# QueensGambit/CrazyAra

Measured on AMD Instinct MI355X. Metric: nn_evals_per_sec, higher is better.
Workload: dtype f16x3; 1 GPU; crazyhouse RISEv2 19-block (34x8x8 planes -> 5184 policy + value), batch=256, inputs resident in HBM, random-init seeded weights; batch=256, parallelism=replicas x1, precision=float16x3

## Files before the change

crazyara_amd/csrc/nn/kernels.h:

```cpp
#pragma once
#include <hip/hip_runtime.h>
#include <cstdint>

namespace cra {

typedef _Float16 half_t;

constexpr int kSquares = 64;

inline int64_t packed_weight_elems(int cout_pad, int k_total) { return int64_t(cout_pad) * k_total; }

struct ConvArgs {
    const void* x;
    const void* wpk;
    const void* wpk_lo;
    const float* bias;
    const void* resid;
    void* out;
    int batch;
    int cin;
    int cout_pad;
    int cout_real;
    int cout_ld;
    int ks;
    int relu;
    int out_policy_f32;
    int out_flat;
    int flat_pitch;
    int out_rows_f32;
    int rows_valid;
    float* softmax_out;
    const float* planes;
    int planes_c;
    int p8;
    float acc_scale;
    const void *pre_wpk, *pre_wpk_lo;
    const float* pre_bias;
    float pre_acc_scale;
    int dev;
    int few_boards;
    int x_ld;
};

template <typename T> void launch_conv_gemm(const ConvArgs& a, hipStream_t s);

struct BlockArgs {
    const void* x;
    void* y;
    const void* w1pk;
    const float* b1;
    const float* wdw;
    const float* b2;
    const void* w3pk;
    const void* w1pk_lo;
    const void* w3pk_lo;
    const float* b3;
    int batch, C, cop_pad, ks;
    const float* gate;
    float* pool_out;
    const float* dwpk;
};
template <typename T> void launch_block(const BlockArgs& a, hipStream_t s);
void launch_conv_gemm_x3(const ConvArgs& a, hipStream_t s);
void launch_block_x3(const BlockArgs& a, hipStream_t s);
void init_x3_kernel_attributes();
int block_x3_chunk_channels();
struct X3TowerBlock {
    const void *w1pk, *w1pk_lo, *w3pk, *w3pk_lo;
    const float* dwpk;
    const float* b3;
    const float* se_w1t;
    const float* se_w2t;
    const float* se_b;
    int cop_pad;
    int se_kind;
    float w1_inv, w3_scale, w3_inv;
    int tail;
};
static_assert(sizeof(X3TowerBlock) == 96, "the tower kernels index a device array of these");
struct X3TowerArgs {
    const float* x;
    float* y;
    const X3TowerBlock* blocks;
    int nblocks;
    int batch;
    int p8;
    int ks;
    int symmetric;
    int no_tail;
    int no_quad;
};
void launch_tower_x3(const X3TowerArgs& a, hipStream_t s);
const char* tower_x3_kernel_name(const X3TowerArgs& a);
void launch_tower_x3_tail(const X3TowerArgs& a, hipStream_t s);
void init_x3_tail_kernel_attributes();
void launch_tower_x3_quad(const X3TowerArgs& a, hipStream_t s);
void init_x3_quad_kernel_attributes();
bool block_x3w_supports(int C, int ks);
void launch_block_x3w(const BlockArgs& a, hipStream_t s);
void init_x3_wblock_kernel_attributes();
void launch_se_gate_w(const float* pool, float* gate, int kind, const float* w1t, const float* w2t, const float* b1, int batch, int C, hipStream_t s);
constexpr int kX3WSplitMaxG = 8;
struct X3WSplitArgs {
    BlockArgs blk;
    const float* x_parts;
    float* y_parts;
    int gin, G;
    int stream_in;
};
int x3w_split_chunks(int cop_pad);
int x3w_split_shares(int cop_pad, int boards, int cu_count);
void launch_block_x3w_split(const X3WSplitArgs& a, hipStream_t s);
void launch_x3w_split_finish(const float* parts, int gin, float* y, float* pool_out, int batch, int C, hipStream_t s);
void init_x3_wsplit_kernel_attributes();
struct X3WTowerBlock {
    const void *w1pk, *w1pk_lo, *w3pk, *w3pk_lo;
    const float* dwpk;
    const float* b3;
    int cop_pad, ks;
};
static_assert(sizeof(X3WTowerBlock) == 56, "tower_x3w_kernel indexes a device array of these");
struct X3WTowerArgs {
    const float* x;
    float* y;
    const X3WTowerBlock* blocks;
    int nblocks;
    const float* gate;
    float* pool_out;
    int batch, C;
};
bool tower_x3w_supports(int C, int ks);
void launch_tower_x3w(const X3WTowerArgs& a, hipStream_t s);
void init_x3_wtower_kernel_attributes();
struct NtbLayer {
    const void *wh, *wl;
    const float* bias;
};
struct NtbArgs {
    const float* x;
    float* y;
    int batch, C, D, M, H;
    NtbLayer patch, qkv, proj, projection, mhca, mhca_proj, mlp1, mlp2;
};
bool ntb_x3w_supports(int C, int D, int M, int H);
void launch_ntb_x3w(const NtbArgs& a, hipStream_t s);
void init_x3_wntb_kernel_attributes();
struct X3SplitArgs {
    X3TowerBlock blk;
    const float* x_parts;
    float* y_parts;
    int gin;
    int batch, G;
    const float* pool_in;
    float* pool_out;
    int dev;
};
void launch_block_x3_split(const X3SplitArgs& a, hipStream_t s);
void launch_x3_split_finish(const float* parts, int gin, float* y, int batch, hipStream_t s);
template <typename T> void init_block_kernel_attributes();
template <typename T> int block_chunk_channels();

constexpr int kTowerWindow = 16;
struct TowerBlockDesc {
    const float* b3;
    const float* s3;
    const void* se_w1;
    const void* se_w2;
    const float* se_b;
    int cop_pad;
    int ks;
    int se_kind;
    float qx_inv, qt_inv, escale;
};
struct TowerArgs {
    const void* x;
    void* y;
    const TowerBlockDesc* blocks;
    const void* wstream;
    const float* bstream;
    const void* pstream;
    long long wstream_wave_frags, bstream_wave_floats, pstream_wave_bytes;
    int nblocks;
    int batch;
    const float* gate_in;
    float* pool_out;
    unsigned long long* trace;
    int fp8;
    long long wstream_e_frags;
    void* block_dump;
};
void launch_tower(const TowerArgs& a, hipStream_t s);
void init_tower_kernel_attributes();
size_t tower_lds_bytes();
inline int tower_row_of_position(int p) { return (p % 4) + 8 * ((p % 16) / 4) + 4 * (p / 16); }
inline int tower_k_channel(int kpos) {
    const int chunk = kpos / 128, wq = (kpos % 128) / 32, p = kpos % 32;
    return chunk * 128 + wq * 32 + tower_row_of_position(p);
}

struct StemArgs {
    const float* planes;
    void* x;
    const void* stem_w;
    const float* stem_b;
    long long stem_wave_frags;
    int cin, cin_pad;
    int batch;
    const void* descs;
    int layout, n_valid;
};
void launch_stem(const StemArgs& a, hipStream_t s);

struct HeadArgs {
    const void* x;
    float* logits;
    float* probs;
    float* value;
    float* aux;
    const void* s1;
    const float* b1;
    const void* s2;
    long long s1_wave_frags, s2_wave_frags;
    const float* vconv_bias;
    const void* fc1_w;
    const float* fc1_b;
    const float* fc2_w;
    float fc2_b;
    float wdl_b[4];
    int cp;
    int wdlp;
    int batch;
    unsigned long long* trace;
    const uint16_t* g_idx;
    const uint32_t* g_cnt;
    float* g_out;
    int g_stride, g_n_valid;
};
void launch_head(const HeadArgs& a, hipStream_t s);
void init_head_kernel_attributes();
size_t head_lds_bytes();

void launch_forward(const StemArgs& sa, const TowerArgs& ta, const HeadArgs& ha, hipStream_t s);
void init_forward_kernel_attributes();

struct ResTowerArgs {
    const void* x;
    void* y;
    const void* wstream;
    const float* bstream;
    long long wstream_wave_frags;
    long long bstream_wave_floats;
    int nblocks;
    int relu_after_add;
    int batch;
    int boards_per_workgroup;
    int cout_tiles_per_wave;
};
void launch_restower(const ResTowerArgs& a, hipStream_t s);
void init_restower_kernel_attributes();
size_t restower_lds_bytes();

template <typename T> void launch_depthwise(const T* x, T* y, const float* w, const float* bias, int batch, int C, int ks,
                                            hipStream_t s);

template <typename T> void launch_se(T* x, int kind_flags, const float* w1t, const float* w2t, const float* b1, int batch, int C,
                                     hipStream_t s, const T* res = nullptr);

void launch_se_gate(const float* pool, float* gate, int kind, const float* w1t, const float* w2t, const float* b1, int batch, int C,
                    hipStream_t s);

struct ValueHeadArgs {
    const void* x;
    const float* wconv;
    const float* bconv;
    const float* w1t;
    const float* b1;
    const float* w2;
    float b2;
    const float* wwdl;
    const float* bwdl;
    const float* wplys;
    float bplys;
    float* value;
    float* aux;
    int batch, C, cv, fc;
    float* dbg;
    int lds_pad;
    int variant;
};
template <typename T> void prepare_value_head(const ValueHeadArgs& a);
size_t value_head_lds_bytes(const ValueHeadArgs& a);
template <typename T> void launch_value_head(const ValueHeadArgs& a, hipStream_t s);

struct HeadsSmallArgs {
    ConvArgs conv;
    ValueHeadArgs vh;
};
bool heads_small_fits(const ConvArgs& c, const ValueHeadArgs& v);
void launch_heads_small(const HeadsSmallArgs& a, hipStream_t s);

struct ValueFinalArgs {
    const void* in;
    int n;
    const float* w;
    float b[4];
    int wdlp;
    float* value;
    float* aux;
    int batch;
};
template <typename T> void launch_value_final(const ValueFinalArgs& a, hipStream_t s);

void launch_gather_probs(const float* probs, int nb_policy, const uint16_t* idx, const uint32_t* cnt, int stride, int n_slots, float* out,
                         const float* value_dev, float* value_out, int batch, const float* aux_dev, float* aux_out, hipStream_t s);

void launch_gather_probs_indexed(const float* probs, int nb_policy, const uint16_t* idx, const uint32_t* cnt, int stride, const int* board_of,
                                 int n_slots, float* out, const float* value_dev, float* value_out, const float* aux_dev, float* aux_out,
                                 hipStream_t s);
void launch_scatter_rows_indexed(const float* probs, const float* logits, int nb_policy, const int* board_of, int n_slots, float* probs_out,
                                 float* logits_out, const float* value_dev, float* value_out, const float* aux_dev, float* aux_out, hipStream_t s);
void launch_gather_planes_indexed(const float* src, const int* board_of, int n_slots, int row, float* dst, hipStream_t s);

struct AttentionArgs {
    const void* qkv;
    void* out;
    int batch;
    int D;
    int mode;
};
void launch_attention(const AttentionArgs& a, hipStream_t s);

void launch_softmax(const float* logits, float* probs, int batch, int n, hipStream_t s);

template <typename T> void launch_planes_to_act(const float* planes, T* act, int batch, int C, int cpad, hipStream_t s);

}
```

crazyara_amd/csrc/nn/precision.cpp:

```cpp
#include <cstdlib>
#include <stdexcept>

#include "rise_net.h"

namespace cra {

namespace {
constexpr bool kX3ValueHeadOneLaunch = true;
}

RiseNet::DevSwitches::DevSwitches() {
    if (const char* e = getenv("CRA_X3_CONV_DEV")) conv_dev = atoi(e);
    device_graph = getenv("CRA_DEVICE_GRAPH") != nullptr;
    lane_graph = getenv("CRA_LANE_GRAPH") != nullptr;
    lane_no_graph = getenv("CRA_LANE_NO_GRAPH") != nullptr;
    predict_copy = getenv("CRA_PREDICT_COPY") != nullptr;
    predict_zero_copy = getenv("CRA_PREDICT_ZERO_COPY") != nullptr;
    if (const char* e = getenv("CRA_LANE_LAUNCHES")) lane_launches = e[0];
    lane_sync = getenv("CRA_LANE_SYNC") != nullptr;
    if (const char* e = getenv("CRA_X3_TOWER")) x3_symmetric = e[0] == 's';
    if (const char* e = getenv("CRA_X3_SPLIT_DEV")) x3_split_dev = atoi(e);
    no_small_path = getenv("CRA_NO_SMALL_PATH") != nullptr;
    if (const char* e = getenv("CRA_SMALL_BATCH_CONV_SPLIT")) small_conv_split = atoi(e);
    tower_trace = getenv("CRA_TOWER_TRACE") != nullptr;
    x3_value_one_launch = kX3ValueHeadOneLaunch;
    if (const char* e = getenv("CRA_X3_VALUE_HEAD")) x3_value_one_launch = e[0] == 'o';
    value_head_debug = getenv("CRA_VALUE_HEAD_DEBUG") != nullptr;
    if (const char* e = getenv("CRA_VALUE_HEAD_LDS_PAD")) value_head_lds_pad = atoi(e);
    if (const char* e = getenv("CRA_VALUE_HEAD_VARIANT")) value_head_variant = atoi(e);
    x3_no_head_chain = getenv("CRA_X3_NO_HEAD_CHAIN") != nullptr;
    x3_no_tail = getenv("CRA_X3_NO_TAIL") != nullptr;
    x3_no_quad = getenv("CRA_X3_NO_QUAD") != nullptr;
    small_batch_heads_apart = getenv("CRA_SMALL_BATCH_HEADS_APART") != nullptr;
    if (const char* e = getenv("CRA_X3_HEADS_APART")) x3_heads_apart = e[0] != '0' && e[0] != 0;
    value_head_env = getenv("CRA_X3_VALUE_HEAD") != nullptr || getenv("CRA_VALUE_HEAD_VARIANT") != nullptr;
}

Precision parse_precision(const std::string& precision) {
    Precision v;
    std::string prec = precision;
    auto strip = [&](const std::string& tag) {
        if (prec.size() <= tag.size() || prec.compare(prec.size() - tag.size(), tag.size(), tag) != 0) return false;
        prec.resize(prec.size() - tag.size());
        return true;
    };
    if (strip("-3k")) v.one_launch = false;
    if (strip("-8w")) v.thin_waves = true;
    if (strip("-1wg")) v.board_split = false;
    if (strip("-1b")) v.boards_per_wg = 1;
    else if (strip("-2b")) v.boards_per_wg = 2;
    if (strip("-wtower")) v.wtower = v.wnet = v.wblock = true;
    else if (strip("-wsplit")) v.wsplit = v.wnet = v.wblock = true;
    else if (strip("-wnet")) v.wnet = v.wblock = true;
    else if (strip("-wblock")) v.wblock = true;
    if (strip("-unfused")) v.fused = v.tower = false;
    else if (strip("-perblock")) v.tower = false;
    using M = Precision::Mode;
    static const std::pair<const char*, M> kModes[] = {
        {"float16", M::Float16},   {"fp16", M::Float16},     {"half", M::Float16},      {"int8", M::Int8},
        {"fp8", M::Fp8},           {"float8", M::Fp8},       {"float32", M::Float32},   {"fp32", M::Float32},
        {"float16x3", M::Float16x3}, {"fp16x3", M::Float16x3}, {"f16x3", M::Float16x3},
        {"float16p8", M::Float16p8}, {"fp16p8", M::Float16p8}, {"f16p8", M::Float16p8}};
    for (const auto& m : kModes)
        if (prec == m.first) {
            v.mode = m.second;
            if (v.wtower && !v.x3()) throw std::invalid_argument("`-wtower` is a float16x3 kernel family (float16x3-wtower | float16p8-wtower), got '" + precision + "'");
            if (v.wtower && !v.fused) throw std::invalid_argument("`-wtower` and `-unfused` exclude each other, got '" + precision + "'");
            if (v.wsplit && !v.x3()) throw std::invalid_argument("`-wsplit` is a float16x3 kernel family (float16x3-wsplit | float16p8-wsplit), got '" + precision + "'");
            if (v.wsplit && !v.fused) throw std::invalid_argument("`-wsplit` and `-unfused` exclude each other, got '" + precision + "'");
            if (v.wsplit && !v.board_split)
                throw std::invalid_argument("`-wsplit` and `-1wg` exclude each other (several workgroups per board against one), got '" + precision + "'");
            if (v.wnet && !v.x3()) throw std::invalid_argument("`-wnet` is a float16x3 kernel family (float16x3-wnet | float16p8-wnet), got '" + precision + "'");
            if (v.wnet && !v.fused) throw std::invalid_argument("`-wnet` and `-unfused` exclude each other, got '" + precision + "'");
            if (v.wblock && !v.x3()) throw std::invalid_argument("`-wblock` is a float16x3 kernel family (float16x3-wblock | float16p8-wblock), got '" + precision + "'");
            if (v.wblock && !v.fused) throw std::invalid_argument("`-wblock` and `-unfused` exclude each other, got '" + precision + "'");
            return v;
        }
    throw std::invalid_argument("unsupported precision '" + precision + "' (float16 | float16x3 | float16p8 | float32 | fp8 | int8)");
}

}
```

crazyara_amd/csrc/nn/rise_net.h:

```cpp
#pragma once
#include <hip/hip_runtime.h>
#include <memory>
#include <string>
#include <utility>
#include <vector>

#include "board_net.h"
#include "netfile.h"

namespace cra {

uint8_t float_to_e4m3(float v);
uint8_t float_to_e5m2(float v);

struct Precision {
    enum class Mode { Float32, Float16, Float16x3, Float16p8, Fp8, Int8 };
    Mode mode = Mode::Float16;
    bool fused = true;
    bool tower = true;
    bool one_launch = true;
    bool thin_waves = false;
    bool board_split = true;
    bool wblock = false;
    bool wnet = false;
    bool wsplit = false;
    bool wtower = false;
    int boards_per_wg = 0;
    bool fp16() const { return mode == Mode::Float16 || mode == Mode::Fp8 || mode == Mode::Int8; }
    bool x3() const { return mode == Mode::Float16x3 || mode == Mode::Float16p8; }
    bool p8() const { return mode == Mode::Float16p8; }
    bool fp8_tower() const { return mode == Mode::Fp8 || mode == Mode::Int8; }
    bool int8() const { return mode == Mode::Int8; }
};
Precision parse_precision(const std::string& precision);

class RiseNet : public BoardNet {
public:
    RiseNet(const std::string& model_path, int device_id, int batch_size, const std::string& precision) : RiseNet(model_path, device_id, batch_size, precision, nullptr) {}
    ~RiseNet() override;

    const std::string& model_file_path() const { return model_file_path_; }
    bool fp16() const { return prec_.fp16(); }
    int cu_count() const { return cu_count_; }

    void predict(const float* in_planes, float* value, float* probs, float* aux);
    void submit(const float* in_planes, float* value, float* probs, float* aux);
    void wait() override;
    void submit_boards(const void* descs_host, int n_valid, int layout, float* value, float* probs, float* aux, int routing = -1) override;
    void submit_boards_gathered(const void* descs_host, int n_valid, int layout, const uint16_t* idx, const uint32_t* cnt, uint32_t stride,
                                float* value, float* gathered, float* aux, int routing = -1) override;
    struct Group {
        const int* board_of = nullptr;
        int n = 0;
        int layout = 0;
        const void* descs = nullptr;
        const float* planes = nullptr;
        const uint16_t* idx = nullptr;
        const uint32_t* cnt = nullptr;
        uint32_t stride = 0;
        float* gathered = nullptr;
        float* probs = nullptr;
        float* logits = nullptr;
        float* value = nullptr;
        float* aux = nullptr;
    };
    void run_group(const Group& g);

    std::vector<std::pair<float, float>> calibration_maxima(const float* planes_host, int n_boards);

    void keep_logits(bool on) override;
    void* enable_block_dump(int* n_tiles);
    void dev_launch_op(int op, int iters);
    float* value_head_debug() const { return value_head_dbg_; }
    int dev_screen_prepare();
    long dev_screen_run(int op, int launches, long* words);
    std::string dev_screen_info(int op) const;
    void forward_async();

    int launches_per_forward() const { return launches_; }
    const char* op_name(int i) const;
    const char* op_kernel(int i) const;
    void time_ops(int iters, float* ms);
    float time_forward(int iters);

    struct IoOverride {
        const float* planes = nullptr;
        float* value = nullptr;
        float* probs = nullptr;
        float* aux = nullptr;
    };
    bool last_submit_was_zero_copy() const { return last_zero_copy_; }

private:
    friend class ExpertSet;
    struct ForwardCall {
        int boards = 0;
        const IoOverride* io = nullptr;
        int prev_g = 1;
    };
    RiseNet(const std::string& model_path, int device_id, int batch_size, const std::string& precision, const RiseNet* parent);
    struct Impl;
    template <typename T> struct Builder;
    template <typename T> void build(const NetFile& nf);
    template <typename T> void enqueue(hipStream_t s, ForwardCall call);
    template <typename T> void launch_op(int i, hipStream_t s, ForwardCall& call);
    void launch_forward_in_stream(ForwardCall call);
    void forward_on(hipStream_t s, ForwardCall call);
    int boards_of_call(int n_valid) const;
    void capture();
    bool buffers_are_pinned(const float* in_planes, float* value, float* probs, float* aux);
    bool last_zero_copy_ = false;
    bool counted_in_flight_ = false;
    int staged_calls_left_ = 0;
    struct DevSwitches {
        int conv_dev = -1;
        bool device_graph = false;
        bool lane_graph = false;
        bool lane_no_graph = false;
        bool predict_copy = false;
        bool predict_zero_copy = false;
        char lane_launches = 0;
        bool lane_sync = false;
        bool x3_symmetric = false;
        int x3_split_dev = 0;
        bool no_small_path = false;
        int small_conv_split = 2;
        bool tower_trace = false;
        bool x3_value_one_launch;
        bool value_head_debug = false;
        int value_head_lds_pad = -1;
        int value_head_variant = 0;
        bool x3_no_head_chain = false;
        bool x3_no_tail = false;
        bool x3_no_quad = false;
        bool small_batch_heads_apart = false;
        bool x3_heads_apart = false;
        bool value_head_env = false;
        DevSwitches();
    } dev_;
    float* value_head_dbg_ = nullptr;

    std::string model_file_path_;
    Precision prec_;
    std::vector<std::pair<float, float>> int8_calib_;
    static constexpr int kBoardSplitMaxBatch = 64;
    std::unique_ptr<RiseNet> small_;
    bool owns_stream_ = true;
    int stream_slot_ = -1;
    std::string precision_arg_;
    int cu_count_ = 256;
    int launches_ = 0;
    hipGraph_t graph_ = nullptr;
    hipGraphExec_t graph_exec_ = nullptr;
    void* d_desc_ = nullptr;
    std::unique_ptr<Impl> impl_;
};

std::string int8_calibration_path(const std::string& model_file_path);
std::vector<std::pair<float, float>> read_int8_calibration(const std::string& model_file_path);
std::string calibrate_int8(const std::string& model_path, int device_id, const float* planes_host, int n_boards);
std::vector<float> default_calibration_planes(int channels, int version, int* n_boards);

}
```

crazyara_amd/csrc/nn/rise_net.hip:

```cpp
#include "rise_net.h"

#include <cmath>
#include <cstdio>
#include <cstring>
#include <fstream>
#include <algorithm>

#include "net_streams.h"
#include "onnx_import.h"
#include "rise_net_impl.h"
#include "../chess/planes_host.h"

namespace cra {

RiseNet::RiseNet(const std::string& model_path, int device_id, int batch_size, const std::string& precision, const RiseNet* parent)
    : BoardNet(device_id), impl_(new Impl) {
    if (batch_size <= 0) throw std::invalid_argument("batch size must be positive");
    precision_arg_ = precision;
    prec_ = parse_precision(precision);
    design_.batch = batch_size;

    std::string dir, file;
    auto ends_with = [&](const char* ext) { const size_t n = strlen(ext); return model_path.size() > n && model_path.compare(model_path.size() - n, n, ext) == 0; };
    if (ends_with(".cranet") || ends_with(".onnx")) {
        const size_t sl = model_path.find_last_of('/');
        dir = sl == std::string::npos ? "./" : model_path.substr(0, sl + 1);
        file = sl == std::string::npos ? model_path : model_path.substr(sl + 1);
    } else {
        if (model_path.empty()) throw std::invalid_argument("The given directory must not be empty.");
        dir = model_path.back() == '/' ? model_path : model_path + "/";
        file = find_model_file(dir, batch_size);
    }
    model_name_ = file;
    model_file_path_ = dir + file;
    design_.version = read_version_from_string(model_name_);
    design_.game_phase = read_game_phase_from_string(dir);

    int ndev = 0;
    HIP_CHECK(hipGetDeviceCount(&ndev));
    if (device_id < 0 || device_id >= ndev) throw std::invalid_argument("device id out of range");
    HIP_CHECK(hipSetDevice(device_id));
    {
        int cus = 0;
        if (hipDeviceGetAttribute(&cus, hipDeviceAttributeMultiprocessorCount, device_id) == hipSuccess && cus > 0) cu_count_ = cus;
    }

    NetFile nf;
    if (model_file_path_.size() > 5 && model_file_path_.compare(model_file_path_.size() - 5, 5, ".onnx") == 0) import_onnx(model_file_path_, nf);
    else nf.load(model_file_path_);
    if (nf.str("arch") != "rise") throw std::runtime_error("unsupported arch '" + nf.str("arch") + "' in " + model_file_path_);
    if (parent) {
        stream_ = parent->stream_;
        stream_slot_ = parent->stream_slot_;
        owns_stream_ = false;
    } else {
        stream_ = take_net_stream(device_id, &stream_slot_);
    }
    if (prec_.int8()) {
        int8_calib_ = read_int8_calibration(model_file_path_);
        if (int8_calib_.empty())
            throw std::runtime_error("Precision int8 needs a calibration of this model: " + int8_calibration_path(model_file_path_) +
                                     " is missing -- mi_net_calibrate_int8 makes it (integration/hipapi.h does that with the engine's calibration positions)");
    }
    if (prec_.fp16()) build<half_t>(nf); else build<float>(nf);
    capture();
    if (!dev_.no_small_path && prec_.x3() && prec_.tower && prec_.fused && prec_.board_split && design_.batch > kBoardSplitMaxBatch)
        small_.reset(new RiseNet(model_file_path_, device_id, kBoardSplitMaxBatch, precision_arg_, this));
}

RiseNet::~RiseNet() {
    if (counted_in_flight_) predicts_in_flight(device_)->fetch_sub(1, std::memory_order_relaxed);
    (void)hipSetDevice(device_);
    small_.reset();
    if (stream_) (void)hipStreamSynchronize(stream_);
    if (graph_exec_) (void)hipGraphExecDestroy(graph_exec_);
    if (graph_) (void)hipGraphDestroy(graph_);
    impl_.reset();
    if (owns_stream_) release_net_stream(device_, stream_slot_, stream_);
}

template <typename T> void RiseNet::launch_op(int i, hipStream_t s, ForwardCall& call) {
    Impl& im = *impl_;
    const int n = call.boards;
    const IoOverride* io = call.io;
    const int B = n > 0 ? n : design_.batch;
    const Op& op = im.ops[i];
    auto boards = [&](ConvArgs c) {
        if (n > 0 && c.batch == design_.batch && !c.out_rows_f32) c.batch = n;
        return c;
    };
    const float* planes = io ? io->planes : d_planes_;
    float* value = io ? io->value : d_value_;
    float* probs = io ? io->probs : d_probs_;
    float* aux = (io && d_aux_) ? (io->aux ? io->aux : d_aux_) : d_aux_;
    switch (op.kind) {
        case OpKind::PlanesToAct:
            launch_planes_to_act<T>(op.x == d_planes_ ? planes : static_cast<const float*>(op.x), static_cast<T*>(op.y), B, op.C, im.cin_pad, s);
            break;
        case OpKind::Conv:
            if (op.heads_x3) {
                HeadsX3Args h;
                h.conv = boards(op.conv);
                h.conv.softmax_out = probs;
                if (!keep_logits_) h.conv.out = nullptr;
                h.vh = op.vh;
                h.vh.value = value;
                h.vh.aux = aux;
                h.vh.batch = h.conv.batch;
                launch_heads_x3(h, s);
            } else if (prec_.x3() && dev_.conv_dev >= 0) {
                ConvArgs c = boards(op.conv);
                c.dev = dev_.conv_dev;
                if (op.from_planes) c.planes = planes;
                if (op.fused_softmax) { c.softmax_out = probs; if (!keep_logits_) c.out = nullptr; }
                launch_conv_gemm_x3(c, s);
            } else if (prec_.x3() && op.from_planes) {
                ConvArgs c = boards(op.conv);
                c.planes = planes;
                launch_conv_gemm_x3(c, s);
            } else if (prec_.x3() && op.fused_softmax) {
                ConvArgs c = boards(op.conv);
                c.softmax_out = probs;
                if (!keep_logits_) c.out = nullptr;
                launch_conv_gemm_x3(c, s);
            } else if (prec_.x3()) launch_conv_gemm_x3(boards(op.conv), s);
            else launch_conv_gemm<T>(op.conv, s);
            break;
        case OpKind::Depthwise:
            launch_depthwise<T>(static_cast<const T*>(op.x), static_cast<T*>(op.y), op.w0, op.b0, B, op.C, op.ks, s);
            break;
        case OpKind::SE: launch_se<T>(static_cast<T*>(op.y), op.se_kind, op.w0, op.w1, op.b0, B, op.C, s, static_cast<const T*>(op.x)); break;
        case OpKind::ValueHead: {
            ValueHeadArgs v = op.vh;
            v.value = value;
            v.aux = aux;
            if (n > 0) v.batch = n;
            launch_value_head<T>(v, s);
            break;
        }
        case OpKind::HeadsSmall: {
            HeadsSmallArgs h;
            h.conv = boards(op.conv);
            h.conv.softmax_out = probs;
            if (!keep_logits_) h.conv.out = nullptr;
            h.vh = op.vh;
            h.vh.value = value;
            h.vh.aux = aux;
            h.vh.batch = h.conv.batch;
            launch_heads_small(h, s);
            break;
        }
        case OpKind::Softmax: launch_softmax(d_logits_, probs, B, design_.nb_policy, s); break;
        case OpKind::Block:
            if (prec_.x3()) launch_block_x3(op.blk, s);
            else launch_block<T>(op.blk, s);
            break;
        case OpKind::BlockX3W: {
            BlockArgs a = op.blk;
            a.batch = B;
            launch_block_x3w(a, s);
            break;
        }
        case OpKind::TowerX3W: {
            X3WTowerArgs a = op.wt;
            a.batch = B;
            launch_tower_x3w(a, s);
            break;
        }
        case OpKind::BlockX3WSplit: {
            X3WSplitArgs a = op.ws;
            if (n > 0) {
                a.blk.batch = n;
                a.G = x3w_split_shares(a.blk.cop_pad, n, cu_count_);
                a.gin = a.stream_in ? 1 : call.prev_g;
                call.prev_g = a.G;
            }
            launch_block_x3w_split(a, s);
            break;
        }
        case OpKind::X3WSplitFinish:
            launch_x3w_split_finish(op.ws.x_parts, n > 0 ? call.prev_g : op.ws.gin, static_cast<float*>(op.ws.blk.y), op.ws.blk.pool_out, B, op.ws.blk.C, s);
            break;
        case OpKind::NtbX3W: {
            NtbArgs a = op.ntb;
            a.batch = B;
            launch_ntb_x3w(a, s);
            break;
        }
        case OpKind::ValueFinal: {
            ValueFinalArgs v = op.vf;
            v.value = value;
            v.aux = aux;
            launch_value_final<T>(v, s);
            break;
        }
        case OpKind::Tower: launch_tower(op.tw, s); break;
        case OpKind::Head: {
            HeadArgs h = op.hd;
            h.value = value;
            h.probs = probs;
            h.aux = aux;
            h.logits = keep_logits_ ? d_logits_ : nullptr;
            launch_head(h, s);
            break;
        }
        case OpKind::ResTower: launch_restower(op.rt, s); break;
        case OpKind::TowerX3:
            if (n > 0) {
                X3TowerArgs t = op.tx;
                t.batch = n;
                launch_tower_x3(t, s);
            } else launch_tower_x3(op.tx, s);
            break;
        case OpKind::BlockX3Split:
            if (n > 0) {
                X3SplitArgs a = op.xs;
                a.batch = n;
                a.G = std::max(1, std::min(std::min(10, cu_count_ / n), a.blk.cop_pad / block_x3_chunk_channels()));
                a.gin = (i == 0 || im.ops[i - 1].kind != OpKind::BlockX3Split) ? 1 : call.prev_g;
                call.prev_g = a.G;
                launch_block_x3_split(a, s);
            } else launch_block_x3_split(op.xs, s);
            break;
        case OpKind::X3SplitFinish: launch_x3_split_finish(op.xs.x_parts, n > 0 ? call.prev_g : op.xs.gin, op.xs_y, B, s); break;
        case OpKind::Stem: {
            StemArgs st = op.st;
            st.planes = planes;
            launch_stem(st, s);
            break;
        }
        case OpKind::Forward: {
            StemArgs st = op.st;
            HeadArgs h = op.hd;
            st.planes = planes;
            h.value = value;
            h.probs = probs;
            h.aux = aux;
            h.logits = keep_logits_ ? d_logits_ : nullptr;
            launch_forward(st, op.tw, h, s);
            break;
        }
        case OpKind::Attention: {
            AttentionArgs at{op.x, op.y, B, op.C, prec_.fp16() ? 0 : prec_.x3() ? 2 : 1};
            launch_attention(at, s);
            break;
        }
        case OpKind::SEGate:
            if (op.C == 256) launch_se_gate(static_cast<const float*>(op.x), static_cast<float*>(op.y), op.se_kind, op.w0, op.w1, op.b0, B, op.C, s);
            else launch_se_gate_w(static_cast<const float*>(op.x), static_cast<float*>(op.y), op.se_kind, op.w0, op.w1, op.b0, B, op.C, s);
            break;
    }
}

template <typename T> void RiseNet::enqueue(hipStream_t s, ForwardCall call) {
    call.prev_g = 1;
    for (int i = 0; i < int(impl_->ops.size()); ++i) launch_op<T>(i, s, call);
    HIP_CHECK(hipGetLastError());
}

const char* RiseNet::op_name(int i) const {
    const Op& op = impl_->ops.at(i);
    switch (op.kind) {
        case OpKind::PlanesToAct: return "planes_to_act";
        case OpKind::Conv: return prec_.x3() ? (op.conv.ks == 1 ? "conv_gemm_x3_1x1" : "conv_gemm_x3_3x3") : (op.conv.ks == 1 ? "conv_gemm_1x1" : "conv_gemm_3x3");
        case OpKind::Depthwise: return "depthwise";
        case OpKind::SE: return "se";
        case OpKind::ValueHead: return "value_head";
        case OpKind::Softmax: return "softmax";
        case OpKind::Block: return prec_.x3() ? "block_x3" : "fused_block";
        case OpKind::ValueFinal: return "value_final";
        case OpKind::SEGate: return "se_gate";
        case OpKind::Tower: return "tower";
        case OpKind::Head: return "head";
        case OpKind::ResTower: return "restower";
        case OpKind::Stem: return "stem";
        case OpKind::Forward: return "forward";
        case OpKind::TowerX3: return op.tx.p8 ? "tower_p8" : "tower_x3";
        case OpKind::BlockX3Split: return "block_x3_split";
        case OpKind::X3SplitFinish: return "x3_split_finish";
        case OpKind::HeadsSmall: return "heads_small";
        case OpKind::Attention: return "attention";
        case OpKind::BlockX3W: return "block_x3w";
        case OpKind::NtbX3W: return "ntb_x3w";
        case OpKind::TowerX3W: return "tower_x3w";
        case OpKind::BlockX3WSplit: return "block_x3w_split";
        case OpKind::X3WSplitFinish: return "x3w_split_finish";
    }
    return "?";
}

const char* RiseNet::op_kernel(int i) const {
    const Op& op = impl_->ops.at(i);
    if (op.kind == OpKind::Conv && op.heads_x3) return kHeadsX3KernelName;
    if (op.kind == OpKind::Conv && prec_.x3() && !op.conv.p8 && op.conv.pre_wpk) return "conv3x3_x3_chain_kernel";
    return op.kind == OpKind::TowerX3 ? tower_x3_kernel_name(op.tx) : op_name(i);
}

void RiseNet::time_ops(int iters, float* ms) {
    HIP_CHECK(hipSetDevice(device_));
    hipEvent_t e0, e1;
    HIP_CHECK(hipEventCreate(&e0));
    HIP_CHECK(hipEventCreate(&e1));
    const int n = int(impl_->ops.size());
    for (int it = 0; it < iters; ++it)
        for (int i = 0; i < n; ++i) {
            HIP_CHECK(hipEventRecord(e0, stream_));
            ForwardCall call;
            if (prec_.fp16()) launch_op<half_t>(i, stream_, call); else launch_op<float>(i, stream_, call);
            HIP_CHECK(hipEventRecord(e1, stream_));
            HIP_CHECK(hipEventSynchronize(e1));
            float t = 0.f;
            HIP_CHECK(hipEventElapsedTime(&t, e0, e1));
            ms[i] += t;
        }
    (void)hipEventDestroy(e0);
    (void)hipEventDestroy(e1);
    for (const Op& op : impl_->ops)
        if ((op.kind == OpKind::Head || op.kind == OpKind::Forward) && op.hd.trace) {
            unsigned long long h[16];
            HIP_CHECK(hipMemcpy(h, op.hd.trace, sizeof(h), hipMemcpyDeviceToHost));
            fprintf(stderr, "head trace (load, conv1, pack, conv2, atomics, softmax, value):");
            for (int i = 1; i < 8; ++i) fprintf(stderr, " %llu", h[i] - h[i - 1]);
            fprintf(stderr, "\n");
        }
    for (const Op& op : impl_->ops)
        if ((op.kind == OpKind::Tower || op.kind == OpKind::Forward) && op.tw.trace) {
            std::vector<unsigned long long> h(512);
            HIP_CHECK(hipMemcpy(h.data(), op.tw.trace, 512 * sizeof(unsigned long long), hipMemcpyDeviceToHost));
            for (int wv = 0; wv < 2; ++wv) {
                fprintf(stderr, "tower trace wave %d:", wv * 4);
                for (int i = 1; i < 256 && h[wv * 256 + i]; ++i) fprintf(stderr, " %llu", h[wv * 256 + i] - h[wv * 256 + i - 1]);
                fprintf(stderr, "\n");
            }
        }
}

namespace {
__global__ __launch_bounds__(256) void screen_compare_kernel(const uint4* __restrict__ a, const uint4* __restrict__ b, size_t n16, unsigned* bad) {
    unsigned diff = 0;
    for (size_t i = size_t(blockIdx.x) * 256 + threadIdx.x; i < n16; i += size_t(gridDim.x) * 256) {
        const uint4 x = a[i], y = b[i];
        diff += (x.x != y.x || x.y != y.y || x.z != y.z || x.w != y.w) ? 1u : 0u;
    }
    if (diff) atomicAdd(bad, diff);
}
void screen_compare(const char* a, const char* b, size_t bytes, unsigned* bad, hipStream_t s) {
    const size_t n16 = bytes / 16;
    if (!n16) return;
    const int blocks = int(std::min<size_t>(512, (n16 + 255) / 256));
    hipLaunchKernelGGL(screen_compare_kernel, dim3(blocks), dim3(256), 0, s, reinterpret_cast<const uint4*>(a), reinterpret_cast<const uint4*>(b), n16, bad);
}
}

int RiseNet::dev_screen_prepare() {
    HIP_CHECK(hipSetDevice(device_));
    Impl& im = *impl_;
    if (!im.screen.empty()) return int(im.screen.size());
    auto salloc = [&](size_t bytes) {
        void* p = nullptr;
        HIP_CHECK(hipMalloc(&p, bytes ? bytes : 16));
        im.screen_allocs.push_back(p);
        return static_cast<char*>(p);
    };
    im.screen_bad = reinterpret_cast<unsigned*>(salloc(sizeof(unsigned) * 65536));
    unsigned* flag = reinterpret_cast<unsigned*>(salloc(sizeof(unsigned) * im.mutables.size()));
    std::vector<char*> snap(im.mutables.size());
    for (size_t i = 0; i < im.mutables.size(); ++i) snap[i] = salloc(im.mutables[i].second);
    HIP_CHECK(hipStreamSynchronize(stream_));
    im.screen.resize(im.ops.size());
    std::vector<unsigned> hflag(im.mutables.size());
    for (int k = 0; k < int(im.ops.size()); ++k) {
        for (size_t i = 0; i < im.mutables.size(); ++i)
            HIP_CHECK(hipMemcpyAsync(snap[i], im.mutables[i].first, im.mutables[i].second, hipMemcpyDeviceToDevice, stream_));
        HIP_CHECK(hipMemsetAsync(flag, 0, sizeof(unsigned) * im.mutables.size(), stream_));
        dev_launch_op(k, 1);
        for (size_t i = 0; i < im.mutables.size(); ++i) screen_compare(snap[i], im.mutables[i].first, im.mutables[i].second, flag + i, stream_);
        HIP_CHECK(hipMemcpyAsync(hflag.data(), flag, sizeof(unsigned) * hflag.size(), hipMemcpyDeviceToHost, stream_));
        HIP_CHECK(hipStreamSynchronize(stream_));
        ScreenOp& so = im.screen[k];
        for (size_t i = 0; i < im.mutables.size(); ++i) {
            if (!hflag[i]) continue;
            ScreenOp::Buf b{im.mutables[i].first, salloc(im.mutables[i].second), salloc(im.mutables[i].second), im.mutables[i].second};
            HIP_CHECK(hipMemcpyAsync(b.before, snap[i], b.bytes, hipMemcpyDeviceToDevice, stream_));
            HIP_CHECK(hipMemcpyAsync(b.after, b.live, b.bytes, hipMemcpyDeviceToDevice, stream_));
            so.writes.push_back(b);
        }
        HIP_CHECK(hipMemsetAsync(flag, 0, sizeof(unsigned), stream_));
        dev_launch_op(k, 1);
        for (const ScreenOp::Buf& b : so.writes) screen_compare(b.after, b.live, b.bytes, flag, stream_);
        HIP_CHECK(hipMemcpyAsync(hflag.data(), flag, sizeof(unsigned), hipMemcpyDeviceToHost, stream_));
        HIP_CHECK(hipStreamSynchronize(stream_));
        so.idempotent = hflag[0] == 0;
        if (!so.idempotent)
            for (const ScreenOp::Buf& b : so.writes) HIP_CHECK(hipMemcpyAsync(b.live, b.after, b.bytes, hipMemcpyDeviceToDevice, stream_));
        HIP_CHECK(hipStreamSynchronize(stream_));
    }
    return int(im.screen.size());
}

long RiseNet::dev_screen_run(int op, int launches, long* words) {
    HIP_CHECK(hipSetDevice(device_));
    Impl& im = *impl_;
    if (im.screen.empty()) throw std::runtime_error("dev_screen_run: dev_screen_prepare first");
    if (op < 0 || op >= int(im.screen.size())) throw std::invalid_argument("op index out of range");
    launches = std::min(launches, 65536);
    const ScreenOp& so = im.screen[op];
    HIP_CHECK(hipMemsetAsync(im.screen_bad, 0, sizeof(unsigned) * launches, stream_));
    for (int l = 0; l < launches; ++l) {
        if (!so.idempotent)
            for (const ScreenOp::Buf& b : so.writes) HIP_CHECK(hipMemcpyAsync(b.live, b.before, b.bytes, hipMemcpyDeviceToDevice, stream_));
        dev_launch_op(op, 1);
        for (const ScreenOp::Buf& b : so.writes) screen_compare(b.after, b.live, b.bytes, im.screen_bad + l, stream_);
        if ((l & 63) == 63) HIP_CHECK(hipStreamSynchronize(stream_));
    }
    std::vector<unsigned> bad(launches);
    HIP_CHECK(hipMemcpyAsync(bad.data(), im.screen_bad, sizeof(unsigned) * launches, hipMemcpyDeviceToHost, stream_));
    HIP_CHECK(hipStreamSynchronize(stream_));
    long n = 0, w = 0;
    for (unsigned b : bad) { n += b != 0; w += b; }
    if (words) *words = w;
    return n;
}

std::string RiseNet::dev_screen_info(int op) const {
    const Impl& im = *impl_;
    if (op < 0 || op >= int(im.screen.size())) return "";
    size_t bytes = 0;
    for (const ScreenOp::Buf& b : im.screen[op].writes) bytes += b.bytes;
    return std::string(op_name(op)) + " writes " + std::to_string(im.screen[op].writes.size()) + " buffers / " + std::to_string(bytes) + " bytes" +
           (im.screen[op].idempotent ? "" : ", not idempotent (buffers restored before every launch)");
}

void RiseNet::dev_launch_op(int op, int iters) {
    HIP_CHECK(hipSetDevice(device_));
    if (op < 0 || op >= int(impl_->ops.size())) throw std::invalid_argument("op index out of range");
    ForwardCall call;
    for (int it = 0; it < iters; ++it) {
        if (prec_.fp16()) launch_op<half_t>(op, stream_, call); else launch_op<float>(op, stream_, call);
    }
    HIP_CHECK(hipGetLastError());
}

float RiseNet::time_forward(int iters) {
    HIP_CHECK(hipSetDevice(device_));
    hipEvent_t e0, e1;
    HIP_CHECK(hipEventCreate(&e0));
    HIP_CHECK(hipEventCreate(&e1));
    HIP_CHECK(hipEventRecord(e0, stream_));
    for (int it = 0; it < iters; ++it) HIP_CHECK(hipGraphLaunch(graph_exec_, stream_));
    HIP_CHECK(hipEventRecord(e1, stream_));
    HIP_CHECK(hipEventSynchronize(e1));
    float t = 0.f;
    HIP_CHECK(hipEventElapsedTime(&t, e0, e1));
    (void)hipEventDestroy(e0);
    (void)hipEventDestroy(e1);
    return t;
}

void RiseNet::keep_logits(bool on) {
    if (on == keep_logits_) return;
    keep_logits_ = on;
    if (launches_ > 1 && graph_exec_) {
        HIP_CHECK(hipStreamSynchronize(stream_));
        (void)hipGraphExecDestroy(graph_exec_);
        if (graph_) (void)hipGraphDestroy(graph_);
        graph_exec_ = nullptr;
        graph_ = nullptr;
        capture();
    }
}

void RiseNet::capture() {
    hipStream_t cs = nullptr;
    HIP_CHECK(hipStreamCreateWithFlags(&cs, hipStreamNonBlocking));
    hipError_t err = hipStreamBeginCapture(cs, hipStreamCaptureModeThreadLocal);
    if (err != hipSuccess) {
        (void)hipStreamDestroy(cs);
        HIP_CHECK(err);
    }
    try {
        forward_on(cs, ForwardCall{});
    } catch (...) {
        hipGraph_t g = nullptr;
        (void)hipStreamEndCapture(cs, &g);
        if (g) (void)hipGraphDestroy(g);
        (void)hipStreamDestroy(cs);
        throw;
    }
    err = hipStreamEndCapture(cs, &graph_);
    (void)hipStreamDestroy(cs);
    HIP_CHECK(err);
    HIP_CHECK(hipGraphInstantiate(&graph_exec_, graph_, nullptr, nullptr, 0));
}

void RiseNet::forward_on(hipStream_t s, ForwardCall call) {
    if (prec_.fp16()) enqueue<half_t>(s, call); else enqueue<float>(s, call);
}

void RiseNet::forward_async() {
    touch_net_stream(device_, stream_slot_);
    Turn turn(device_, design_.batch, cu_count_, stream_);
    if (launches_ == 1 && !dev_.device_graph) {
        forward_on(stream_, ForwardCall{});
        HIP_CHECK(hipGetLastError());
        return;
    }
    HIP_CHECK(hipGraphLaunch(graph_exec_, stream_));
}

void RiseNet::launch_forward_in_stream(ForwardCall call) {
    touch_net_stream(device_, stream_slot_);
    Turn turn(device_, design_.batch, cu_count_, stream_);
    if (call.boards > 0 || (launches_ <= 5 && !dev_.lane_graph) || dev_.lane_no_graph) forward_on(stream_, call);
    else HIP_CHECK(hipGraphLaunch(graph_exec_, stream_));
}
// ... 247 lines not shown
```

crazyara_amd/csrc/nn/rise_net_build.hip:

```cpp
#include <algorithm>
#include <cmath>
#include <cstring>
#include <type_traits>

#include "../chess/planes_host.h"
#include "pack.h"
#include "rise_net_impl.h"

namespace cra {

namespace {
enum class Family {
    Tower,
    X3Tower,
    X3Split,
    Fused,
    WBlock,
    WSplit,
    WTower,
    Layers,
    Transformer,
    WNtb
};
struct BlockPlan {
// ... 426 lines not shown
            ba.b3 = im.upload_d2f(bf.project.b, C);
            ba.batch = B;
            ba.C = C;
            ba.cop_pad = cop_pad;
            ba.ks = k;
            if (k == 3)
                ba.dwpk = im.upload(prec.x3() ? pack_x3_depthwise_records(bf.expand, bf.dw, cop, cop_pad, 3)
                                             : pack_depthwise_records12(bf.expand, bf.dw, cop, cop_pad));
            ba.gate = pending_gate;
            pending_gate = nullptr;
            prod_op = int(im.ops.size());
            im.ops.push_back(op);
            std::swap(cur, nxt);
        } else if (bp.family == Family::WBlock) {
            const int cop_pad = round_up(cop, 64);
            const X3BlockPack pk = pack_x3_block(fold_block(nf, p), C, cop, k, cop_pad, false);
            Op op;
            op.kind = OpKind::BlockX3W;
            BlockArgs& ba = op.blk;
            ba.x = cur;
            ba.y = nxt;
            ba.w1pk = im.upload(pk.w1.hi);
            ba.w1pk_lo = im.upload(pk.w1.lo);
            ba.w3pk = im.upload(pk.w3.hi);
            ba.w3pk_lo = im.upload(pk.w3.lo);
            ba.dwpk = im.upload(pk.dw);
            ba.b3 = im.upload(pk.b3);
            ba.batch = B;
            ba.C = C;
            ba.cop_pad = cop_pad;
            ba.ks = k;
            ba.gate = pending_gate;
            pending_gate = nullptr;
            prod_op = int(im.ops.size());
            im.ops.push_back(op);
            ++wblock_ops;
            std::swap(cur, nxt);
        } else if (bp.family == Family::WTower) {
            const int cop_pad = round_up(cop, 64);
            const X3BlockPack pk = pack_x3_block(fold_block(nf, p), C, cop, k, cop_pad, false);
            BlockArgs ba{};
            ba.w1pk = im.upload(pk.w1.hi);
            ba.w1pk_lo = im.upload(pk.w1.lo);
            ba.w3pk = im.upload(pk.w3.hi);
            ba.w3pk_lo = im.upload(pk.w3.lo);
            ba.dwpk = im.upload(pk.dw);
            ba.b3 = im.upload(pk.b3);
            ba.batch = B;
            ba.C = C;
            ba.cop_pad = cop_pad;
            ba.ks = k;
            ba.gate = pending_gate;
            pending_gate = nullptr;
            wrun.push_back(ba);
            ++wblock_ops;
        } else if (bp.family == Family::WSplit) {
            const int cop_pad = round_up(cop, 64);
            const X3BlockPack pk = pack_x3_block(fold_block(nf, p), C, cop, k, cop_pad, false);
            if (!wsplit_parts[0]) {
                int max_chunks = 1;
                for (size_t q = 0; q < cops.size(); ++q)
                    if (!ntb[q]) max_chunks = std::max(max_chunks, x3w_split_chunks(round_up(cops[q], 64)));
                const size_t images = size_t(std::min(max_chunks, int(kX3WSplitMaxG)));
                for (auto& q : wsplit_parts) q = static_cast<float*>(im.dalloc(size_t(B) * images * kSquares * C * sizeof(float)));
            }
            Op op;
            op.kind = OpKind::BlockX3WSplit;
            BlockArgs& ba = op.ws.blk;
            ba.w1pk = im.upload(pk.w1.hi);
            ba.w1pk_lo = im.upload(pk.w1.lo);
            ba.w3pk = im.upload(pk.w3.hi);
            ba.w3pk_lo = im.upload(pk.w3.lo);
            ba.dwpk = im.upload(pk.dw);
            ba.b3 = im.upload(pk.b3);
            ba.batch = B;
            ba.C = C;
            ba.cop_pad = cop_pad;
            ba.ks = k;
            ba.gate = pending_gate;
            pending_gate = nullptr;
            op.ws.stream_in = wsplit_g == 0 ? 1 : 0;
            op.ws.x_parts = wsplit_g == 0 ? reinterpret_cast<const float*>(cur) : wsplit_parts[wsplit_set];
            op.ws.gin = std::max(1, wsplit_g);
            wsplit_set ^= 1;
            op.ws.y_parts = wsplit_parts[wsplit_set];
            op.ws.G = x3w_split_shares(cop_pad, B, net.cu_count_);
            wsplit_g = op.ws.G;
            prod_op = -1;
            im.ops.push_back(op);
            ++wblock_ops;
        } else {
            add_conv(p + ".body.0", p + ".body.1", cur, e, nullptr, C, C, cop, 1, true, nullptr);
            {
                Folded fd = fold_bn(nf, p + ".body.3", p + ".body.4");
                Op op;
                op.kind = OpKind::Depthwise;
                op.x = e;
                op.y = f;
                op.w0 = im.upload(pack_depthwise_taps(fd, cop, k, cop));
                op.b0 = im.upload_d2f(fd.b);
                op.C = cop;
                op.ks = k;
                im.ops.push_back(op);
                macs += double(kSquares) * cop * k * k;
            }
            add_conv(p + ".body.6", p + ".body.7", f, nxt, cur, cop, cop, C, 1, false, nullptr);
            std::swap(cur, nxt);
            prod_op = -1;
            continue;
        }
        macs += double(kSquares) * cop * (2.0 * C + k * k);
    }
    flush_tower();
    flush_x3_run();
    wsplit_finish();
    flush_wrun();
}

template <typename T> void RiseNet::Builder<T>::flush_wrun() {
    if (wrun.empty()) return;
    Op op;
    if (wrun.size() == 1) {
        op.kind = OpKind::BlockX3W;
        op.blk = wrun[0];
        op.blk.x = cur;
        op.blk.y = nxt;
    } else {
        std::vector<X3WTowerBlock> recs;
        for (const BlockArgs& ba : wrun) {
            if (ba.gate && &ba != &wrun[0]) throw std::logic_error("flush_wrun: a gated block inside a run");
            recs.push_back(X3WTowerBlock{ba.w1pk, ba.w1pk_lo, ba.w3pk, ba.w3pk_lo, ba.dwpk, ba.b3, ba.cop_pad, ba.ks});
        }
        op.kind = OpKind::TowerX3W;
        op.wt.x = reinterpret_cast<const float*>(cur);
        op.wt.y = reinterpret_cast<float*>(nxt);
        op.wt.blocks = im.upload(recs);
        op.wt.nblocks = int(recs.size());
        op.wt.gate = wrun[0].gate;
        op.wt.batch = B;
        op.wt.C = C;
    }
    prod_op = int(im.ops.size());
    im.ops.push_back(op);
    wrun.clear();
    std::swap(cur, nxt);
}

template <typename T> void RiseNet::Builder<T>::wsplit_finish() {
    if (wsplit_g == 0) return;
    Op fin;
    fin.kind = OpKind::X3WSplitFinish;
    fin.ws.x_parts = wsplit_parts[wsplit_set];
    fin.ws.gin = wsplit_g;
    fin.ws.blk.y = cur;
    fin.ws.blk.C = C;
    fin.ws.blk.batch = B;
    prod_op = int(im.ops.size());
    im.ops.push_back(fin);
    wsplit_g = 0;
}

template <typename T> void RiseNet::Builder<T>::transformer_block(size_t i) {
    const NtbFold n = fold_ntb(nf, "body_spatial." + std::to_string(i + 1), C);
    const int D = n.D, M = n.M, H = n.H;
    T* xs = nxt;
    conv_op(n.patch, cur, xs, C, C, D, 1, 0).cout_ld = C;
    conv_op(n.qkv, xs, e, D, D, 3 * D, 1, 0).x_ld = C;
    {
        Op op;
        op.kind = OpKind::Attention;
        op.x = e;
        op.y = f;
        op.C = D;
        im.ops.push_back(op);
    }
    {
        ConvArgs& c = conv_op(n.proj, f, xs, D, D, D, 1, 0);
        c.resid = xs;
        c.cout_ld = C;
    }
    {
        ConvArgs& c = conv_op(n.projection, xs, xs + D, D, D, M, 1, 0);
        c.x_ld = C;
        c.cout_ld = C;
    }
    conv_op(n.mhca, xs + D, f, M, M, M, 3, 1).x_ld = C;
    {
        ConvArgs& c = conv_op(n.mhca_proj, f, xs + D, M, M, M, 1, 0);
        c.resid = xs + D;
        c.cout_ld = C;
    }
    conv_op(n.mlp1, xs, e, C, C, H, 1, 1);
    conv_op(n.mlp2, e, cur, H, H, C, 1, 0).resid = xs;
    macs += n.macs;
    prod_op = -1;
}

template <typename T> void RiseNet::Builder<T>::transformer_block_x3w(const NtbFold& n) {
    const X3NtbPack pk = pack_x3_ntb(n);
    Op op;
    op.kind = OpKind::NtbX3W;
    NtbArgs& a = op.ntb;
    a.x = reinterpret_cast<const float*>(cur);
    a.y = reinterpret_cast<float*>(nxt);
    a.batch = B;
    a.C = C;
    a.D = n.D;
    a.M = n.M;
    a.H = n.H;
    auto layer = [&](const SplitPack& sp, const Folded& fd, int co) { return NtbLayer{im.upload(sp.hi), im.upload(sp.lo), im.upload_d2f(fd.b, size_t(co))}; };
    a.patch = layer(pk.patch, n.patch, n.D);
    a.qkv = layer(pk.qkv, n.qkv, 3 * n.D);
    a.proj = layer(pk.proj, n.proj, n.D);
    a.projection = layer(pk.projection, n.projection, n.M);
    a.mhca = layer(pk.mhca, n.mhca, n.M);
    a.mhca_proj = layer(pk.mhca_proj, n.mhca_proj, n.M);
    a.mlp1 = layer(pk.mlp1, n.mlp1, n.H);
    a.mlp2 = layer(pk.mlp2, n.mlp2, C);
    im.ops.push_back(op);
    macs += n.macs;
    ++wntb_ops;
    prod_op = -1;
    std::swap(cur, nxt);
}

template <typename T> void RiseNet::Builder<T>::flush_tower() {
    if (tower_blocks.empty()) return;
    Op op;
    op.kind = OpKind::Tower;
    op.tw.x = cur;
    op.tw.y = nxt;
    op.tw.blocks = im.upload(tower_blocks);
    op.tw.nblocks = int(tower_blocks.size());
    const TowerImage ti = close_tower_streams(std::move(tower_streams), prec.fp8_tower());
    tower_streams = TowerStreams();
    if (prec.fp8_tower()) {
        op.tw.fp8 = prec.int8() ? 2 : 1;
        op.tw.wstream_e_frags = ti.e_frags;
        op.tw.wstream = im.upload(ti.w8);
    } else {
        op.tw.wstream = im.upload(ti.w);
    }
    op.tw.bstream = im.upload(ti.b);
    op.tw.pstream = im.upload(ti.p);
    op.tw.wstream_wave_frags = ti.w_wave_frags;
    op.tw.bstream_wave_floats = ti.b_wave_floats;
    op.tw.pstream_wave_bytes = ti.p_wave_bytes;
    op.tw.batch = B;
    op.tw.gate_in = tower_gate;
    if (dev.tower_trace) op.tw.trace = static_cast<unsigned long long*>(im.dalloc(2 * 256 * sizeof(unsigned long long)));
    prod_op = int(im.ops.size());
    im.ops.push_back(op);
    tower_blocks.clear();
    tower_gate = nullptr;
    std::swap(cur, nxt);
}

template <typename T> void RiseNet::Builder<T>::flush_x3_run() {
    if (x3_blocks.empty()) return;
    if (x3_split && x3_run_ks == 3) {
        if (!split_parts[0])
            for (auto& q : split_parts) q = static_cast<float*>(im.dalloc(size_t(B) * kSplitMaxG * kSquares * C * sizeof(float)));
        const int max_g = std::max(1, std::min(int(kSplitMaxG), net.cu_count_ / B));
        const int nb = int(x3_blocks.size());
        int gin = 1;
        for (int k = 0; k < nb; ++k) {
            Op op;
            op.kind = OpKind::BlockX3Split;
            op.xs.blk = x3_blocks[k];
            op.xs.x_parts = k == 0 ? reinterpret_cast<const float*>(cur) : split_parts[k % 2];
            op.xs.y_parts = split_parts[(k + 1) % 2];
            op.xs.gin = gin;
            op.xs.batch = B;
            op.xs.G = std::min(max_g, x3_blocks[k].cop_pad / block_x3_chunk_channels());
            op.xs.dev = dev.x3_split_dev;
            if (k > 0 && x3_blocks[k].se_kind != 0 && !(dev.x3_split_dev & 8)) {
                float* pools = static_cast<float*>(im.dalloc(size_t(B) * kSplitMaxG * C * sizeof(float)));
                im.ops.back().xs.pool_out = pools;
                op.xs.pool_in = pools;
            }
            gin = op.xs.G;
            im.ops.push_back(op);
        }
        Op fin;
        fin.kind = OpKind::X3SplitFinish;
        fin.xs.x_parts = split_parts[nb % 2];
        fin.xs.gin = gin;
        fin.xs.batch = B;
        fin.xs_y = reinterpret_cast<float*>(nxt);
        im.ops.push_back(fin);
    } else {
        Op op;
        op.kind = OpKind::TowerX3;
        op.tx.x = reinterpret_cast<const float*>(cur);
        op.tx.y = reinterpret_cast<float*>(nxt);
        op.tx.blocks = im.upload(x3_blocks);
        op.tx.nblocks = int(x3_blocks.size());
        op.tx.batch = B;
        op.tx.p8 = prec.p8() ? 1 : 0;
        op.tx.ks = x3_run_ks;
        op.tx.symmetric = dev.x3_symmetric ? 1 : 0;
        op.tx.no_tail = dev.x3_no_tail ? 1 : 0;
        op.tx.no_quad = dev.x3_no_quad ? 1 : 0;
        im.ops.push_back(op);
    }
    x3_blocks.clear();
    prod_op = -1;
    std::swap(cur, nxt);
}

template <typename T> void RiseNet::Builder<T>::one_launch_head() {
    const Folded fv = fold_bn(nf, "value_head.body.0", "value_head.body.1");
    const HeadStreams hs = pack_head(fold_bn(nf, "policy_head.body.0", "policy_head.body.1"), fold_bn(nf, "policy_head.body.3", ""), fv, C, cv, cp);
    Op op;
    op.kind = OpKind::Head;
    HeadArgs& h = op.hd;
    h.x = cur;
    h.logits = net.d_logits_;
    h.probs = net.d_probs_;
    h.value = net.d_value_;
    h.aux = net.d_aux_;
    h.s1 = im.upload(hs.s1);
    h.b1 = im.upload(hs.b1);
    h.s2 = im.upload(hs.s2);
    h.s1_wave_frags = 9 * 16 + 16 + 16;
    h.s2_wave_frags = 18 * 3 + 9;
    h.vconv_bias = im.upload_d2f(fv.b, 8);
    h.cp = cp;
    h.batch = B;
    if (dev.tower_trace) h.trace = static_cast<unsigned long long*>(im.dalloc(64 * sizeof(unsigned long long)));
    const int nfl = kSquares * cv;
    if (wdl) {
        h.fc1_w = im.upload(pack_value_wdl(nf, nfl, 512));
        const float* bw = nf.get("value_head.body_wdl.0.bias").data;
        h.wdl_b[0] = bw[0]; h.wdl_b[1] = bw[1]; h.wdl_b[2] = bw[2];
        h.wdl_b[3] = nf.get("value_head.body_plys.0.bias").data[0];
        h.wdlp = 1;
        macs += 4.0 * nfl;
    } else {
        const TensorView& w2 = nf.get("value_head.body_final.2.weight");
        const float* bb = nf.get("value_head.body_final.0.bias").data;
        h.fc1_w = im.upload(pack_value_fc1_threads(nf, nfl, fc));
        h.fc1_b = im.upload(std::vector<float>(bb, bb + fc));
        h.fc2_w = im.upload(std::vector<float>(w2.data, w2.data + fc));
        h.fc2_b = nf.get("value_head.body_final.2.bias").data[0];
        macs += double(nfl) * fc + fc;
    }
    macs += double(kSquares) * 9 * (double(C) * C + double(C) * cp) + double(kSquares) * C * cv;
    im.ops.push_back(op);
}

template <typename T> void RiseNet::Builder<T>::policy_head() {
    const bool head_chain = prec.p8() && policy_map && C == 256 && round_up(cp, 16) <= 128 && !x3_split;
    const bool head_chain_x3 = prec.x3() && !prec.p8() && prec.fused && policy_map && C == 256 && round_up(cp, 16) <= 128 && !x3_split &&
                               !dev.x3_no_head_chain;
    if (head_chain || head_chain_x3) {
        Folded f1 = fold_bn(nf, "policy_head.body.0", "policy_head.body.1");
        double inv1 = 1.0;
        SplitPack s1 = head_chain ? pack_dense_p8(f1, C, C, 3, C, C, &inv1) : pack_dense_split(f1, C, C, 3, C, C);
        add_conv("policy_head.body.3", "", cur, nullptr, nullptr, C, C, cp, 3, false, net.d_logits_, head_chain);
        ConvArgs& c = im.ops.back().conv;
        c.pre_wpk = im.upload(s1.hi);
        c.pre_wpk_lo = im.upload(s1.lo);
        c.pre_bias = im.upload_d2f(f1.b, C);
        c.pre_acc_scale = float(inv1);
        macs += double(kSquares) * C * C * 9;
        return;
    }
    add_conv("policy_head.body.0", "policy_head.body.1", cur, nxt, nullptr, C, C, C, 3, true, nullptr, !x3_split);
    im.ops.back().conv.few_boards = x3_split ? dev.small_conv_split : 0;
    if (policy_map) {
        add_conv("policy_head.body.3", "", nxt, nullptr, nullptr, C, C, cp, 3, false, net.d_logits_, !x3_split);
        return;
    }
    const int nfl = cp * kSquares, Bpad = round_up(B, 64);
    T* pflat = static_cast<T*>(im.dalloc(size_t(Bpad) * nfl * sizeof(T)));
    HIP_CHECK(hipMemset(pflat, 0, size_t(Bpad) * nfl * sizeof(T)));
    ConvArgs& c1 = conv_op(fold_bn(nf, "policy_head.body.3", "policy_head.body2.0"), nxt, pflat, C, C, cp, 3, 1);
    c1.out_flat = 1;
    c1.flat_pitch = nfl;
    macs += double(kSquares) * C * cp * 9;
    const TensorView& w = nf.get("policy_head.body3.0.weight");
    const float* bb = nf.get("policy_head.body3.0.bias").data;
    Folded fl;
    fl.w.assign(w.data, w.data + size_t(n_labels) * nfl);
    fl.b.assign(bb, bb + n_labels);
    ConvArgs& c2 = conv_op(fl, pflat, net.d_logits_, nfl, nfl, n_labels, 1, 0);
    c2.batch = Bpad / 64;
    c2.out_rows_f32 = 1;
    c2.rows_valid = B;
    macs += double(nfl) * n_labels;
}

template <typename T> void RiseNet::Builder<T>::softmax() {
    if (prec.x3() && !im.ops.empty() && im.ops.back().kind == OpKind::Conv && im.ops.back().conv.out_policy_f32 &&
        im.ops.back().conv.cout_pad <= 256 && im.ops.back().conv.cout_real * kSquares <= 8192) {
        im.ops.back().fused_softmax = true;
    } else {
        Op op;
        op.kind = OpKind::Softmax;
        im.ops.push_back(op);
    }
}

template <typename T> void RiseNet::Builder<T>::value_head() {
    const bool x3_value_one_launch = prec.x3() && prec.fused && dev.x3_value_one_launch;
    const int nfl = kSquares * cv;
    if (prec.fused && !x3_value_one_launch) {
        const int Bpad = round_up(B, 64);
        T* vflat = static_cast<T*>(im.dalloc(size_t(Bpad) * nfl * sizeof(T)));
        HIP_CHECK(hipMemset(vflat, 0, size_t(Bpad) * nfl * sizeof(T)));
        ConvArgs& c = conv_op(fold_bn(nf, "value_head.body.0", "value_head.body.1"), cur, vflat, C, C, cv, 1, 1);
        c.out_flat = 1;
        c.flat_pitch = nfl;
        macs += double(kSquares) * C * cv;
        Op fin;
        fin.kind = OpKind::ValueFinal;
        ValueFinalArgs& vf = fin.vf;
        vf.value = net.d_value_;
        vf.aux = net.d_aux_;
        vf.batch = B;
        if (wdl) {
            const float* bw = nf.get("value_head.body_wdl.0.bias").data;
            vf.in = vflat;
            vf.n = nfl;
            vf.w = im.upload(pack_value_wdl(nf, nfl, nfl));
            vf.b[0] = bw[0]; vf.b[1] = bw[1]; vf.b[2] = bw[2];
            vf.b[3] = nf.get("value_head.body_plys.0.bias").data[0];
            vf.wdlp = 1;
            macs += 4.0 * nfl;
        } else {
            if (nfl % 32 != 0) throw std::runtime_error("value head flatten size must be a multiple of 32");
            const TensorView &w1 = nf.get("value_head.body_final.0.weight"), &w2 = nf.get("value_head.body_final.2.weight");
            const float* b1 = nf.get("value_head.body_final.0.bias").data;
            Folded f1;
            f1.w.assign(w1.data, w1.data + size_t(fc) * nfl);
            f1.b.assign(b1, b1 + fc);
            const int fc_pad = round_up(fc, 16);
            T* vh = static_cast<T*>(im.dalloc(size_t(Bpad) * fc_pad * sizeof(T)));
            conv_op(f1, vflat, vh, nfl, nfl, fc, 1, 1).batch = Bpad / 64;
            vf.in = vh;
            vf.n = fc_pad;
            std::vector<float> w2p(fc_pad, 0.f);
            std::copy(w2.data, w2.data + fc, w2p.begin());
            vf.w = im.upload(w2p);
            vf.b[0] = nf.get("value_head.body_final.2.bias").data[0];
            vf.wdlp = 0;
            macs += double(nfl) * fc + fc;
        }
        im.ops.push_back(fin);
        return;
    }
    Folded fd = fold_bn(nf, "value_head.body.0", "value_head.body.1");
    Op op;
    op.kind = OpKind::ValueHead;
    ValueHeadArgs& v = op.vh;
    v.x = cur;
    v.wconv = im.upload_d2f(fd.w);
    v.bconv = im.upload_d2f(fd.b);
    v.value = net.d_value_;
    v.aux = net.d_aux_;
    v.batch = B;
    v.C = C;
    v.cv = cv;
    v.fc = fc;
    if (wdl) {
        const TensorView &ww = nf.get("value_head.body_wdl.0.weight"), &wp = nf.get("value_head.body_plys.0.weight");
        v.wwdl = im.upload(std::vector<float>(ww.data, ww.data + 3 * nfl));
        const float* bw = nf.get("value_head.body_wdl.0.bias").data;
        v.bwdl = im.upload(std::vector<float>(bw, bw + 3));
        v.wplys = im.upload(std::vector<float>(wp.data, wp.data + nfl));
        v.bplys = nf.get("value_head.body_plys.0.bias").data[0];
        macs += 4.0 * nfl;
    } else {
        const TensorView& w2 = nf.get("value_head.body_final.2.weight");
        v.w1t = im.upload(pack_value_fc1_transposed(nf, nfl, fc));
        const float* b1 = nf.get("value_head.body_final.0.bias").data;
        v.b1 = im.upload(std::vector<float>(b1, b1 + fc));
        v.w2 = im.upload(std::vector<float>(w2.data, w2.data + fc));
        v.b2 = nf.get("value_head.body_final.2.bias").data[0];
        macs += double(nfl) * fc + fc;
    }
    macs += double(kSquares) * C * cv;
    if (dev.value_head_debug) {
        const size_t dbg_bytes = size_t(B) * ((8 + 1024) + (16 + 3 * 1024)) * sizeof(float);
        v.dbg = static_cast<float*>(im.dalloc(dbg_bytes));
        HIP_CHECK(hipMemset(v.dbg, 0, dbg_bytes));
        net.value_head_dbg_ = v.dbg;
    }
    v.lds_pad = dev.value_head_lds_pad;
    v.variant = dev.value_head_variant;
    prepare_value_head<T>(op.vh);
    im.ops.push_back(op);
}

template <typename T> void RiseNet::Builder<T>::merge_heads_small() {
    std::vector<Op>& ops = im.ops;
    if (x3_split && ops.size() >= 2 && ops.back().kind == OpKind::ValueHead && ops[ops.size() - 2].kind == OpKind::Conv &&
        ops[ops.size() - 2].fused_softmax && heads_small_fits(ops[ops.size() - 2].conv, ops.back().vh) && !dev.small_batch_heads_apart) {
        Op vh = ops.back();
        ops.pop_back();
        Op& op = ops.back();
        op.kind = OpKind::HeadsSmall;
        op.vh = vh.vh;
    }
}

template <typename T> void RiseNet::Builder<T>::merge_heads_x3() {
    std::vector<Op>& ops = im.ops;
    if (!(prec.x3() && !prec.p8() && B > RiseNet::kBoardSplitMaxBatch && !dev.x3_heads_apart && !dev.value_head_env && dev.conv_dev < 0)) return;
    if (ops.size() < 2 || ops.back().kind != OpKind::ValueHead || ops[ops.size() - 2].kind != OpKind::Conv) return;
    const Op& pol = ops[ops.size() - 2];
    if (!pol.fused_softmax || pol.from_planes || !heads_x3_fits(pol.conv, ops.back().vh) || pol.conv.batch != ops.back().vh.batch) return;
    const ValueHeadArgs vh = ops.back().vh;
    ops.pop_back();
    ops.back().heads_x3 = true;
    ops.back().vh = vh;
}

template <typename T> void RiseNet::Builder<T>::merge_forward() {
    std::vector<Op>& ops = im.ops;
    if (prec.one_launch && ops.size() == 3 && ops[0].kind == OpKind::Stem && ops[1].kind == OpKind::Tower && ops[2].kind == OpKind::Head &&
        ops[1].tw.gate_in == nullptr && ops[1].tw.pool_out == nullptr) {
        Op op;
        op.kind = OpKind::Forward;
        op.st = ops[0].st;
        op.tw = ops[1].tw;
        op.hd = ops[2].hd;
        ops.assign(1, op);
        init_forward_kernel_attributes();
    }
}

template <typename T> void RiseNet::build(const NetFile& nf) {
    Builder<T> b(*this, nf);
    b.read_model();
    b.stem();
    if (b.dense_blocks && b.tower_ok) b.dense_tower();
    else if (b.dense_blocks) b.dense_layer_blocks();
    else b.bottleneck_blocks();
    if (prec_.wnet && b.wblock_ops == 0 && b.wntb_ops == 0)
        throw std::runtime_error(std::string(prec_.wtower ? "`-wtower`" : "`-wnet`") + " runs the mobile-bottleneck and transformer blocks of 128 / 192 / 224-channel nets in one launch each: no block of this model qualifies (" +
                                 std::to_string(b.C) + " channels, " + (b.dense_blocks ? "dense residual blocks" : "mobile-bottleneck blocks") +
                                 "); use the precision without the suffix");
    if (prec_.wblock && !prec_.wnet && b.wblock_ops == 0)
        throw std::runtime_error("`-wblock` runs the mobile-bottleneck blocks of 128 / 192 / 224-channel nets in one launch each: no block of this model qualifies (" +
                                 std::to_string(b.C) + " channels, " + (b.dense_blocks ? "dense residual blocks" : "mobile-bottleneck blocks") +
                                 "); use the precision without the suffix");
    if (b.head_ok) {
        b.one_launch_head();
    } else {
        b.policy_head();
        b.softmax();
        b.value_head();
        b.merge_heads_small();
        b.merge_heads_x3();
    }
    init_block_kernel_attributes<T>();
    init_x3_kernel_attributes();
    init_x3_heads_kernel_attributes();
    init_x3_wblock_kernel_attributes();
    init_x3_wsplit_kernel_attributes();
    init_x3_wtower_kernel_attributes();
    init_x3_wntb_kernel_attributes();
    init_tower_kernel_attributes();
    init_restower_kernel_attributes();
    init_head_kernel_attributes();
    b.merge_forward();
    design_.flops_per_position = 2.0 * b.macs;
    launches_ = int(impl_->ops.size());
}

template void RiseNet::build<half_t>(const NetFile& nf);
template void RiseNet::build<float>(const NetFile& nf);

}
```

crazyara_amd/csrc/nn/rise_net_impl.h:

```cpp
#pragma once
#include <stdexcept>
#include <string>
#include <utility>
#include <vector>

#include "kernels.h"
#include "rise_net.h"
#include "x3_heads.h"

namespace cra {

#define HIP_CHECK(expr)                                                                                      \
    do {                                                                                                     \
        hipError_t _e = (expr);                                                                              \
        if (_e != hipSuccess)                                                                                \
            throw std::runtime_error(std::string("HIP error ") + hipGetErrorString(_e) + " at " #expr);      \
    } while (0)

enum class OpKind { PlanesToAct, Conv, Depthwise, SE, ValueHead, Softmax, Block, ValueFinal, SEGate, Tower, Head, Stem, ResTower, Forward, TowerX3, BlockX3Split, X3SplitFinish, HeadsSmall, Attention, BlockX3W, NtbX3W, BlockX3WSplit, X3WSplitFinish, TowerX3W };

struct Op {
    OpKind kind;
    ConvArgs conv{};
    bool from_planes = false;
    bool fused_softmax = false;
    bool heads_x3 = false;
    const void* x = nullptr;
    void* y = nullptr;
    const float *w0 = nullptr, *w1 = nullptr, *b0 = nullptr;
    int C = 0, ks = 0, se_kind = 0;
    ValueHeadArgs vh{};
    BlockArgs blk{};
    NtbArgs ntb{};
    ValueFinalArgs vf{};
    TowerArgs tw{};
    HeadArgs hd{};
    ResTowerArgs rt{};
    StemArgs st{};
    X3TowerArgs tx{};
    X3SplitArgs xs{};
    float* xs_y = nullptr;
    X3WTowerArgs wt{};
    X3WSplitArgs ws{};
};

struct ScreenOp {
    struct Buf { char* live; char* before; char* after; size_t bytes; };
    std::vector<Buf> writes;
    bool idempotent = true;
};

struct RiseNet::Impl {
    std::vector<void*> allocs;
    std::vector<std::pair<char*, size_t>> mutables;
    std::vector<Op> ops;
    std::vector<ScreenOp> screen;
    std::vector<void*> screen_allocs;
    unsigned* screen_bad = nullptr;
    int cin_pad = 0;

    void* dalloc(size_t bytes, bool constant = false) {
        void* p = nullptr;
        HIP_CHECK(hipMalloc(&p, bytes ? bytes : 16));
        allocs.push_back(p);
        if (!constant) mutables.emplace_back(static_cast<char*>(p), bytes ? bytes : 16);
        return p;
    }
    template <typename U> U* upload(const std::vector<U>& h) {
        U* d = static_cast<U*>(dalloc(h.size() * sizeof(U), true));
        HIP_CHECK(hipMemcpy(d, h.data(), h.size() * sizeof(U), hipMemcpyHostToDevice));
        return d;
    }
    float* upload_d2f(const std::vector<double>& h, size_t pad_to = 0) {
        std::vector<float> f(std::max(h.size(), pad_to), 0.f);
        for (size_t i = 0; i < h.size(); ++i) f[i] = float(h[i]);
        return upload(f);
    }
    ~Impl() {
        for (void* p : allocs) (void)hipFree(p);
        for (void* p : screen_allocs) (void)hipFree(p);
    }
};

}
```

crazyara_amd/csrc/nn/x3.hip:

```cpp
#include "kernels.h"
#include "device_utils.h"
#include "value_head_body.h"
#include "x3_device.h"
#include "x3_conv_device.h"

#include <algorithm>
#include <cstdlib>
#include <stdexcept>
#include <type_traits>

#ifndef X3_SGB_VALU
#define X3_SGB_VALU 10
#endif

namespace cra {

namespace {

typedef int i32x4_x3 __attribute__((ext_vector_type(4)));
typedef int i32x8_x3 __attribute__((ext_vector_type(8)));
__device__ __forceinline__ uint32_t x3_high_bytes(uint32_t p01, uint32_t p23) {
    return __builtin_amdgcn_perm(p23, p01, 0x07050301u);
}
__device__ __forceinline__ void split4_b8(const float (&v)[4], half4& hi, uint32_t& h8, uint32_t& l8) {
// ... 1530 lines not shown
                            if (ph == 0) dw.template gather<0, true>(accD[dt], hi, 0, 2, e_inv);
                            if (ph == 1) { dw.template taps<0>(0, 4); dw.pin_taps(0, 4, 0); }
                            if (ph == 2) dw.template gather<1, true>(accD[dt], hi, 0, 2, e_inv);
                            if (ph == 3) dw.template taps<1>(0, 4);
                        } else {
                            if (ph == 0) { dw5.template gather<0>(accD[dt], hi, e_inv); dw5.template taps<0>(); }
                            if (ph == 1) { dw5.template gather<1>(accD[dt], hi, e_inv); dw5.template taps<1>(); }
                            if (ph == 2) { dw5.template gather<2>(accD[dt], hi, e_inv); dw5.template taps<2>(); }
                            if (ph == 3) { dw5.template gather<3>(accD[dt], hi, e_inv); dw5.template taps<3>(); }
                        }
                        if (ph == 3) {
#pragma unroll
                            for (int t = 0; t < 4; ++t) {
                                half4 h;
                                uint32_t h8, l8;
                                split4_b8(KS == 3 ? dw.outv[t] : dw5.outv[t], h, h8, l8);
                                if constexpr ((X3_ABL & 64) != 0) {
                                    asm volatile("" ::"v"(h), "v"(h8), "v"(l8));
                                    continue;
                                }
                                *reinterpret_cast<half4*>(t2h + (t * 16 + l15) * TROW + t2h_col + dt * 16) = h;
                                *reinterpret_cast<uint32_t*>(t2b + (t * 16 + l15) * T8ROW + t2b_col + dt * 32) = h8;
                                *reinterpret_cast<uint32_t*>(t2b + (t * 16 + l15) * T8ROW + T8LO + t2b_col + dt * 32) = l8;
                            }
                        }
                    }
                    if constexpr (HASE && HASD) {
#pragma unroll
                        for (int r = 0; r < 16; ++r) {
                            __builtin_amdgcn_sched_group_barrier(0x008, 1, 0);
                            __builtin_amdgcn_sched_group_barrier(0x002, KS == 3 ? X3_SGB_VALU : 12, 0);
                        }
                    }
                    __builtin_amdgcn_sched_barrier(0);
                }
                if constexpr (HASE) {
#pragma unroll
                    for (int ne = 0; ne < 2; ++ne)
#pragma unroll
                        for (int h2 = 0; h2 < REC / 256; ++h2) *reinterpret_cast<f32x4*>(my_dws + ne * REC + h2 * 256 + lane * 4) = dw_raw[ne][h2];
#pragma unroll
                    for (int ne = 0; ne < 2; ++ne)
#pragma unroll
                        for (int t = 0; t < 4; ++t) accD[ne][t] = accE[ne][t];
                }
            };
            for (int i = 0; i <= n; ++i) {
                const int kk = i - 1;
                X3_STAMP(0);
                if (i == 0) interval(std::true_type{}, std::false_type{}, i);
                else if (i < n) interval(std::true_type{}, std::true_type{}, i);
                else interval(std::false_type{}, std::true_type{}, i);
                X3_STAMP(3);
                __syncthreads();
                X3_STAMP(4);
            }
            __syncthreads();
            { const int kk = n; X3_STAMP(5); }
        }
        return;
    }

    f32x4 accX[NJ][4];
    {
        const float* xb = a.x + size_t(b) * 64 * C;
#pragma unroll
        for (int j = 0; j < NJ; ++j)
#pragma unroll
            for (int t = 0; t < 4; ++t)
                accX[j][t] = *reinterpret_cast<const f32x4*>(xb + size_t(x3_square(t * 16 + l15)) * C + (w * NJ + j) * 16 + lg * 4);
    }
    auto write_tiles = [&]() {
#pragma unroll
        for (int j = 0; j < NJ; ++j) {
            const int co0 = (w * NJ + j) * 16 + lg * 4;
#pragma unroll
            for (int t = 0; t < 4; ++t) {
                const int rr = t * 16 + l15;
                float v[4] = {accX[j][t][0], accX[j][t][1], accX[j][t][2], accX[j][t][3]};
                half4 h;
                uint32_t h8, l8;
                split4_b8(v, h, h8, l8);
                const int ch = ((w * 4 + j) * 2 + (lg >> 1)) ^ g0 ^ (g2 << 2);
                const int cb = ((w * 4 + (j & 1) * 2 + (j >> 1)) ^ g0 ^ (g2 << 2)) * 16 + lg * 4;
                *reinterpret_cast<half4*>(T.xh + rr * XROW + ch * 8 + (lg & 1) * 4) = h;
                *reinterpret_cast<uint32_t*>(x8 + rr * X8ROW + cb) = h8;
                *reinterpret_cast<uint32_t*>(x8 + rr * X8ROW + 272 + cb) = l8;
            }
        }
    };
    const half_t* const t2h_even = T.t2h + l15 * TROW + g2 * 32 + (lg ^ g0) * 8;
    const half_t* const t2h_odd = T.t2h + l15 * TROW + (g2 ^ 1) * 32 + (lg ^ g0) * 8;
    const char* const t2b_j0 = t28 + l15 * T8ROW + (lg >> 1) * T8LO + g2 * 64 + (((lg & 1) ^ g0) << 4);
    const char* const t2b_j1 = t28 + l15 * T8ROW + (lg >> 1) * T8LO + (g2 ^ 1) * 64 + (((lg & 1) ^ g0) << 4);
    if (a.blocks[0].se_kind == 0) write_tiles();
    __syncthreads();
    for (int blk = 0; blk < a.nblocks; ++blk) {
        const X3TowerBlock& d = a.blocks[blk];
        if (d.se_kind != 0) {
            constexpr int GRP = 36;
#pragma unroll
            for (int j = 0; j < NJ; ++j) {
                float sum[4];
#pragma unroll
                for (int r = 0; r < 4; ++r) sum[r] = (accX[j][0][r] + accX[j][1][r]) + (accX[j][2][r] + accX[j][3][r]);
#pragma unroll
                for (int r = 0; r < 4; ++r) {
                    sum[r] += dpp_mov<0x111>(sum[r]);
                    sum[r] += dpp_mov<0x112>(sum[r]);
                    sum[r] += dpp_mov<0x114>(sum[r]);
                    sum[r] += dpp_mov<0x118>(sum[r]);
                }
                if (l15 == 15) {
                    const int c = (w * NJ + j) * 16 + lg * 4;
#pragma unroll
                    for (int r = 0; r < 4; ++r) se_scratch[((c + r) >> 5) * GRP + ((c + r) & 31)] = sum[r] * (1.f / 64.f);
                }
            }
            x3_se_gate_from_mean(d, se_scratch, tid);
            const float* se_gate = se_scratch + 12 * GRP;
#pragma unroll
            for (int j = 0; j < NJ; ++j) {
                const f32x4 g = *reinterpret_cast<const f32x4*>(se_gate + (w * NJ + j) * 16 + lg * 4);
#pragma unroll
                for (int t = 0; t < 4; ++t) accX[j][t] *= g;
            }
            write_tiles();
            __syncthreads();
        }
        const X3Weights W = x3_weights(d.w1pk, d.w1pk_lo, d.w3pk, d.w3pk_lo, d.dwpk, d.cop_pad);
        const int n = W.cop_pad / CK;
        const int nslab3 = W.cop_pad >> 5;
#ifdef CRA_X3_TRACE
        const bool tracing = (b == 0 || b == 131) && blk == CRA_X3_TRACE;
        int trace_n = 0;
#endif
        half8 p_h[2][NJ];
        i32x8_x3 p_8[NJ];
        auto load_ph = [&](int k, int s2) {
            if constexpr (X3_ABL & 16) return;
#pragma unroll
            for (int j = 0; j < NJ; ++j) p_h[s2 & 1][j] = x3_frag(W.w3h, lane_off, uint32_t(w * NJ + j) * uint32_t(nslab3) + uint32_t(k * (CK / 32) + s2));
        };
        auto load_p8 = [&](int k, int J) {
#pragma unroll
            for (int j = 0; j < NJ; ++j) {
                const uint32_t f = uint32_t(w * NJ + j) * uint32_t(nslab3) + uint32_t(k * (CK / 32) + 2 * J);
                if constexpr (X3_ABL & (16 | 1024)) continue;
                if constexpr (X3_ABL & 512) {
                    const half8 piece = x3_frag(W.w3l, lane_off, f);
                    p_8[j] = x3_cat(piece, piece);
                    continue;
                }
                p_8[j] = x3_cat(x3_frag(W.w3l, lane_off, f), x3_frag(W.w3l, lane_off, f + 1));
            }
        };
        if constexpr (X3_ABL & (16 | 1024)) {
#pragma unroll
            for (int j = 0; j < NJ; ++j) {
                const half8 any = *reinterpret_cast<const half8*>(T.xh + lane * 8 + j * 512);
                p_8[j] = x3_cat(any, any);
                if constexpr (X3_ABL & 16) p_h[0][j] = p_h[1][j] = any;
            }
        }
        {
            const float ps = d.w3_scale;
#pragma unroll
            for (int j = 0; j < NJ; ++j) {
                const f32x4 bs = *reinterpret_cast<const f32x4*>(d.b3 + (w * NJ + j) * 16 + lg * 4) * ps;
#pragma unroll
                for (int t = 0; t < 4; ++t)
#pragma unroll
                    for (int r = 0; r < 4; ++r) accX[j][t][r] = fmaf(accX[j][t][r], ps, bs[r]);
            }
        }
        load_ph(0, 0);
        load_ph(0, 1);
        load_p8(0, 0);
        __syncthreads();
        __syncthreads();
        for (int kk = 0; kk < n; ++kk) {
            X3_STAMP(8);
            half8 bh[2][4];
            i32x8_x3 b8[4];
            auto read_h = [&](int s2) {
                const half_t* const pe = s2 & 1 ? t2h_odd : t2h_even;
#pragma unroll
                for (int t = 0; t < 4; ++t) bh[s2 & 1][t] = *reinterpret_cast<const half8*>(pe + (kk & 1) * 64 * TROW + t * 16 * TROW + (s2 >> 1) * 64);
            };
            auto read_8 = [&](int J) {
                const char* const pj = J ? t2b_j1 : t2b_j0;
#pragma unroll
                for (int t = 0; t < 4; ++t) {
                    const char* pp = pj + (kk & 1) * 64 * T8ROW + t * 16 * T8ROW;
                    b8[t] = x3_cat(*reinterpret_cast<const half8*>(pp), *reinterpret_cast<const half8*>(pp + 32));
                }
            };
            const int knext = kk + 1 < n ? kk + 1 : kk;
            read_h(0);
            read_8(0);
#pragma unroll
            for (int s2 = 0; s2 < CK / 32; ++s2) {
                if (s2 + 1 < CK / 32) read_h(s2 + 1);
                __builtin_amdgcn_sched_barrier(0);
#pragma unroll
                for (int j = 0; j < NJ; ++j)
#pragma unroll
                    for (int t = 0; t < 4; ++t) x3_mfma(p_h[s2 & 1][j], bh[s2 & 1][t], accX[j][t], !(X3_ABL & 4));
                if (s2 & 1) {
#pragma unroll
                    for (int j = 0; j < NJ; ++j)
#pragma unroll
                        for (int t = 0; t < 4; ++t) x3_mfma8(p_8[j], b8[t], accX[j][t], !(X3_ABL & 4));
                    __builtin_amdgcn_sched_barrier(0);
                    if (s2 == 1) { read_8(1); load_p8(kk, 1); } else load_p8(knext, 0);
                }
                if (s2 + 2 < CK / 32) load_ph(kk, s2 + 2); else load_ph(knext, s2 + 2 - CK / 32);
                __builtin_amdgcn_sched_barrier(0);
            }
            X3_STAMP(10);
            if (kk + 1 < n) __syncthreads();
            X3_STAMP(11);
        }
        {
            const float pi = d.w3_inv;
#pragma unroll
            for (int j = 0; j < NJ; ++j)
#pragma unroll
                for (int t = 0; t < 4; ++t) accX[j][t] *= pi;
        }
        const bool next_gated = blk + 1 < a.nblocks && a.blocks[blk + 1].se_kind != 0;
        if (!next_gated) write_tiles();
        { const int kk = n; X3_STAMP(12); }
        __syncthreads();
        { const int kk = n; X3_STAMP(13); }
    }
    float* yb = a.y + size_t(b) * 64 * C;
#pragma unroll
    for (int j = 0; j < NJ; ++j)
#pragma unroll
        for (int t = 0; t < 4; ++t)
            *reinterpret_cast<f32x4*>(yb + size_t(x3_square(t * 16 + l15)) * C + (w * NJ + j) * 16 + lg * 4) = accX[j][t];
}

void init_x3_kernel_attributes() {
    (void)hipFuncSetAttribute(reinterpret_cast<const void*>(&block_x3_kernel), hipFuncAttributeMaxDynamicSharedMemorySize, int(X3Block::lds_bytes));
    (void)hipFuncSetAttribute(reinterpret_cast<const void*>(&tower_x3_kernel), hipFuncAttributeMaxDynamicSharedMemorySize, int(X3Block::lds_bytes));
    (void)hipFuncSetAttribute(reinterpret_cast<const void*>(&block_x3_split_kernel), hipFuncAttributeMaxDynamicSharedMemorySize, int(X3Block::lds_bytes));
    (void)hipFuncSetAttribute(reinterpret_cast<const void*>(&tower_x3_roles_kernel<3>), hipFuncAttributeMaxDynamicSharedMemorySize, int(X3Block::lds_bytes));
    (void)hipFuncSetAttribute(reinterpret_cast<const void*>(&tower_x3_roles_kernel<5>), hipFuncAttributeMaxDynamicSharedMemorySize, int(X3Block::lds_bytes + 8192));
    init_x3_tail_kernel_attributes();
    init_x3_quad_kernel_attributes();
    (void)hipFuncSetAttribute(reinterpret_cast<const void*>(&tower_p8_kernel<3>), hipFuncAttributeMaxDynamicSharedMemorySize, int(X3Block::lds_bytes));
    (void)hipFuncSetAttribute(reinterpret_cast<const void*>(&tower_p8_kernel<5>), hipFuncAttributeMaxDynamicSharedMemorySize, int(X3Block::lds_bytes + 8192));
    (void)hipFuncSetAttribute(reinterpret_cast<const void*>(&conv3x3_x3_chain_kernel), hipFuncAttributeMaxDynamicSharedMemorySize, int(ConvX3::lds_bytes));
    const int conv_p8_lds = int(ConvP8::lds_bytes);
    (void)hipFuncSetAttribute(reinterpret_cast<const void*>(&conv3x3_p8_chain_kernel), hipFuncAttributeMaxDynamicSharedMemorySize, conv_p8_lds);
    (void)hipFuncSetAttribute(reinterpret_cast<const void*>(&conv3x3_p8_kernel<2, 8>), hipFuncAttributeMaxDynamicSharedMemorySize, conv_p8_lds);
    (void)hipFuncSetAttribute(reinterpret_cast<const void*>(&conv3x3_p8_kernel<1, 8>), hipFuncAttributeMaxDynamicSharedMemorySize, conv_p8_lds);
}
int block_x3_chunk_channels() { return X3Block::CK; }

void launch_block_x3(const BlockArgs& a, hipStream_t s) {
    hipLaunchKernelGGL(block_x3_kernel, dim3(a.batch), dim3(X3Block::NTHR), X3Block::lds_bytes, s, a);
}
void launch_block_x3_split(const X3SplitArgs& a, hipStream_t s) {
    const int n = a.blk.cop_pad / X3Block::CK;
    if (a.G < 1 || a.G > n || a.G > 16 || a.gin < 1 || a.gin > 16) throw std::invalid_argument("block_x3_split: 1 <= G <= min(chunks, 16), 1 <= gin <= 16");
    hipLaunchKernelGGL(block_x3_split_kernel, dim3(8 * a.G * ((a.batch + 7) / 8)), dim3(X3Block::NTHR), X3Block::lds_bytes, s, a);
}
void launch_x3_split_finish(const float* parts, int gin, float* y, int batch, hipStream_t s) {
    const int n4 = batch * 64 * X3Block::C / 4;
    hipLaunchKernelGGL(x3_split_finish_kernel, dim3(std::min(1024, (n4 + 255) / 256)), dim3(256), 0, s, parts, gin, y, batch);
}
namespace {
enum class X3TowerKernel { P8_5, P8_3, Quad3, Tail5, Tail3, Roles5, Roles3, Symmetric };
X3TowerKernel pick_tower_x3(const X3TowerArgs& a) {
    const bool symmetric = a.symmetric != 0;
    if (a.p8) {
        if (symmetric) throw std::invalid_argument("Precision float16p8 runs the two-role tower only");
        return a.ks == 5 ? X3TowerKernel::P8_5 : X3TowerKernel::P8_3;
    }
    if (!symmetric && !a.no_tail) {
        if (a.ks == 5) return X3TowerKernel::Tail5;
        return a.no_quad ? X3TowerKernel::Tail3 : X3TowerKernel::Quad3;
    }
    if (a.ks == 5) return X3TowerKernel::Roles5;
    return symmetric ? X3TowerKernel::Symmetric : X3TowerKernel::Roles3;
}
}
const char* tower_x3_kernel_name(const X3TowerArgs& a) {
    switch (pick_tower_x3(a)) {
        case X3TowerKernel::P8_5: return "tower_p8_kernel<5>";
        case X3TowerKernel::P8_3: return "tower_p8_kernel<3>";
        case X3TowerKernel::Quad3: return "tower_x3_quad_kernel<3>";
        case X3TowerKernel::Tail5: return "tower_x3_tail_kernel<5>";
        case X3TowerKernel::Tail3: return "tower_x3_tail_kernel<3>";
        case X3TowerKernel::Roles5: return "tower_x3_roles_kernel<5>";
        case X3TowerKernel::Roles3: return "tower_x3_roles_kernel<3>";
        case X3TowerKernel::Symmetric: return "tower_x3_kernel";
    }
    return "?";
}
void launch_tower_x3(const X3TowerArgs& a, hipStream_t s) {
    switch (pick_tower_x3(a)) {
        case X3TowerKernel::P8_5: hipLaunchKernelGGL(tower_p8_kernel<5>, dim3(a.batch), dim3(X3Block::NTHR), X3Block::lds_bytes + 8192, s, a); break;
        case X3TowerKernel::P8_3: hipLaunchKernelGGL(tower_p8_kernel<3>, dim3(a.batch), dim3(X3Block::NTHR), X3Block::lds_bytes, s, a); break;
        case X3TowerKernel::Quad3: launch_tower_x3_quad(a, s); break;
        case X3TowerKernel::Tail5:
        case X3TowerKernel::Tail3: launch_tower_x3_tail(a, s); break;
        case X3TowerKernel::Roles5: hipLaunchKernelGGL(tower_x3_roles_kernel<5>, dim3(a.batch), dim3(X3Block::NTHR), X3Block::lds_bytes + 8192, s, a); break;
        case X3TowerKernel::Roles3: hipLaunchKernelGGL(tower_x3_roles_kernel<3>, dim3(a.batch), dim3(X3Block::NTHR), X3Block::lds_bytes, s, a); break;
        case X3TowerKernel::Symmetric: hipLaunchKernelGGL(tower_x3_kernel, dim3(a.batch), dim3(X3Block::NTHR), X3Block::lds_bytes, s, a); break;
    }
}

}
```

crazyara_amd/csrc/nn/x3_quad.cpp:

```cpp
#include "x3_device.h"
#include "x3_quad.h"

#include <type_traits>

namespace cra {

template <int KS>
__global__ __launch_bounds__(512) void tower_x3_quad_kernel(const X3TowerArgs a) {
    static_assert(KS == 3, "depthwise 3x3 (X3DepthwiseQuad); 5x5 runs stay on tower_x3_tail_kernel");
    constexpr int REC = 256;
    using G = X3Block;
    static_assert(G::NE == 1 && G::T2BUF == 2 && G::CK == 128, "the role kernel uses the NE = 1 tile geometry (two t2 buffers of 128 channels)");
    static_assert(X3Q_T2T_HALVES <= 64 * G::TROW, "t2T of a chunk lies in the [64][TROW] tile's place");
    constexpr int C = G::C, CK = G::CK, XROW = G::XROW, TROW = G::TROW;
    extern __shared__ __attribute__((aligned(16))) char smem[];
    const X3Tiles T = x3_tiles(smem);
    const int b = blockIdx.x;
    const int tid = threadIdx.x, lane = tid & 63, l15 = lane & 15, lg = lane >> 4;
    const int wave = __builtin_amdgcn_readfirstlane(tid >> 6);
    const bool expand_role = wave < 4;
    const int w = wave & 3;
    const uint32_t lane_off = uint32_t(lane) * 16u;
    x3_stage_tile(T, a.x + size_t(b) * 64 * C, nullptr, tid);
    __syncthreads();
    constexpr int EW = 2;
    half8 e_h[EW][2], e_l[EW][2];
    bool first_chunk_requested = false;
    if (expand_role) {
    for (int blk = 0; blk < a.nblocks; ++blk) {
        const X3TowerBlock& d = a.blocks[blk];
        if (blk > 0 && d.se_kind != 0) {
            x3_se_gate_from_mean(d, reinterpret_cast<float*>(T.t2h), tid);
            __syncthreads();
            first_chunk_requested = false;
#pragma unroll
            for (int ne = 0; ne < 2; ++ne) {
#pragma unroll
                for (int q = 0; q < EW; ++q) { asm volatile("" : "=v"(e_h[q][ne])); asm volatile("" : "=v"(e_l[q][ne])); }
            }
        }
        const X3Weights W = x3_weights(d.w1pk, d.w1pk_lo, d.w3pk, d.w3pk_lo, d.dwpk, d.cop_pad);
        const int n = W.cop_pad / CK;
        const bool tail = __builtin_amdgcn_readfirstlane(d.tail) != 0;
#ifdef CRA_X3_TRACE
        const bool tracing = (b == 0 || b == 131) && blk == CRA_X3_TRACE;
        int trace_n = 0;
#endif
        {
            const X3QuadOffsets qo = x3_quad_offsets(lane);
            int sto[4];
#pragma unroll
            for (int t = 0; t < 4; ++t) sto[t] = x3q_store_offset(0, l15, lg, t);
            auto e_tile = [&](int i, int ne) { return i * (CK / 16) + (tail && i == n - 1 ? w : w * 2 + ne); };
            auto load_e = [&](auto one_c, int i, int s) {
                if constexpr (X3_ABL & 16) return;
#pragma unroll
                for (int ne = 0; ne < (decltype(one_c)::value ? 1 : 2); ++ne) {
                    const uint32_t f = uint32_t(e_tile(i, ne)) * (C / 32) + uint32_t(s);
                    e_h[s % EW][ne] = x3_frag(W.w1h, lane_off, f);
                    e_l[s % EW][ne] = x3_frag(W.w1l, lane_off, f);
                }
            };
            auto load_first_chunk = [&](const X3Weights& Wx, bool one) {
                if constexpr (X3_ABL & 16) return;
#pragma unroll
                for (int s = 0; s < EW; ++s)
#pragma unroll
                    for (int ne = 0; ne < 2; ++ne) {
                        const uint32_t f = uint32_t(one ? w : w * 2 + ne) * (C / 32) + uint32_t(s);
                        e_h[s][ne] = x3_frag(Wx.w1h, lane_off, f);
                        e_l[s][ne] = x3_frag(Wx.w1l, lane_off, f);
                    }
            };
            if constexpr (X3_ABL & 16) {
#pragma unroll
                for (int s = 0; s < EW; ++s)
#pragma unroll
                    for (int ne = 0; ne < 2; ++ne) e_h[s][ne] = e_l[s][ne] = *reinterpret_cast<const half8*>(T.xh + lane * 8);
            }
            if (!first_chunk_requested) load_first_chunk(W, tail && n == 1);
            float* const my_dws = T.dws + (w * 2) * REC;
            f32x4 accE[2][4], accD[2][4];
            X3DepthwiseQuad dw;
            auto interval = [&](auto hase_c, auto hasd_c, auto onee_c, auto oned_c, int i) {
                constexpr bool HASE = decltype(hase_c)::value, HASD = decltype(hasd_c)::value;
                constexpr bool ONEE = decltype(onee_c)::value, ONED = decltype(oned_c)::value;
                static_assert(!(ONEE && !HASE) && !(ONED && (HASE || !HASD)), "the tail chunk is expanded in interval n - 1 and runs the depthwise alone in interval n");
                constexpr int NEE = ONEE ? 1 : 2;
                half8 ring_h[4], ring_l[4];
                auto read_step = [&](int st) {
                    if constexpr (X3_ABL & 8) {
                        ring_h[st % 4] = e_h[0][0];
                        ring_l[st % 4] = e_l[0][0];
                    } else {
                        ring_h[st % 4] = *reinterpret_cast<const half8*>(T.xh + ((st & 3) * 16 + l15) * XROW + (st >> 2) * 32 + lg * 8);
                        ring_l[st % 4] = *reinterpret_cast<const half8*>(T.xl + ((st & 3) * 16 + l15) * XROW + (st >> 2) * 32 + lg * 8);
                    }
                };
                f32x4 dw_raw[NEE][REC / 256];
                if constexpr (HASE) {
#pragma unroll
                    for (int ne = 0; ne < NEE; ++ne)
#pragma unroll
                        for (int h2 = 0; h2 < REC / 256; ++h2)
                            dw_raw[ne][h2] = __builtin_bit_cast(f32x4, __builtin_amdgcn_raw_buffer_load_b128(W.dw, lane_off, uint32_t(e_tile(i, ne) * 16) * uint32_t(REC / 4) + uint32_t(h2) * 1024u, 0));
#pragma unroll
                    for (int ne = 0; ne < NEE; ++ne)
#pragma unroll
                        for (int t = 0; t < 4; ++t) accE[ne][t] = f32x4{0.f, 0.f, 0.f, 0.f};
                    read_step(0); read_step(1); read_step(2);
                }
                if constexpr (HASD) dw.load(my_dws, l15, qo);
                half_t* const t2h = T.t2h + ((i - 1) & 1) * 64 * TROW;
                half_t* const t2l = T.t2l + ((i - 1) & 1) * 64 * TROW;
#pragma unroll
                for (int sl = 0; sl < (ONED ? C / 64 : C / 32); ++sl) {
                    const int dt = sl / 4, ph = sl % 4;
                    if constexpr (HASD) {
                        if (!ONED && sl == 3) dw.load(my_dws + 256, l15, qo);
                    }
                    __builtin_amdgcn_sched_barrier(0);
                    if constexpr (HASE) {
#pragma unroll
                        for (int t = 0; t < 4; ++t) {
                            const int st = sl * 4 + t;
                            if (st + 3 < 4 * (C / 32)) read_step(st + 3);
#pragma unroll
                            for (int ne = 0; ne < NEE; ++ne) {
                                x3_mfma(ring_h[st % 4], e_l[sl % EW][ne], accE[ne][t], !(X3_ABL & 2));
                                x3_mfma(ring_l[st % 4], e_h[sl % EW][ne], accE[ne][t], !(X3_ABL & 2));
                                x3_mfma(ring_h[st % 4], e_h[sl % EW][ne], accE[ne][t], !(X3_ABL & 2));
                            }
                        }
                        if (sl + EW < C / 32) load_e(onee_c, i, sl + EW);
                        else if constexpr (ONEE) load_e(onee_c, i, sl + EW - C / 32);
                        else load_e(onee_c, i + 1 < n ? i + 1 : i, sl + EW - C / 32);
                    }
                    if constexpr (HASD) {
                        if (ph == 0) dw.gather(accD[dt], lg, qo);
                        if (ph == 1) { dw.template taps_rank<0>(); dw.template taps_rank<1>(); dw.template pin_rank<0>(); dw.template pin_rank<1>(); }
                        if (ph == 2) { dw.template taps_rank<2>(); dw.template taps_rank<3>(); dw.template pin_rank<2>(); dw.template pin_rank<3>(); }
                        if (ph == 3) {
                            const int tile = ONED ? w : w * 2 + dt;
#pragma unroll
                            for (int t = 0; t < 4; ++t) {
                                half4 h, l;
                                split4(dw.outv[t], h, l);
                                if constexpr (X3_ABL & 64) {
                                    asm volatile("" ::"v"(h), "v"(l));
                                } else {
                                    *reinterpret_cast<half4*>(t2h + tile * 16 * X3Q_T2T_ROW + sto[t]) = h;
                                    *reinterpret_cast<half4*>(t2l + tile * 16 * X3Q_T2T_ROW + sto[t]) = l;
                                }
                            }
                        }
                    }
                    if constexpr (HASE && HASD) {
#pragma unroll
                        for (int r = 0; r < 12 * NEE; ++r) {
                            __builtin_amdgcn_sched_group_barrier(0x008, 1, 0);
                            __builtin_amdgcn_sched_group_barrier(0x002, ONEE ? 8 : 4, 0);
                        }
                    }
                    __builtin_amdgcn_sched_barrier(0);
                }
                if constexpr (HASE) {
#pragma unroll
                    for (int ne = 0; ne < NEE; ++ne)
#pragma unroll
                        for (int h2 = 0; h2 < REC / 256; ++h2) *reinterpret_cast<f32x4*>(my_dws + ne * REC + h2 * 256 + lane * 4) = dw_raw[ne][h2];
#pragma unroll
                    for (int ne = 0; ne < NEE; ++ne)
#pragma unroll
                        for (int t = 0; t < 4; ++t) accD[ne][t] = accE[ne][t];
                }
            };
            constexpr std::true_type yes{};
            constexpr std::false_type no{};
            auto run = [&](auto hase_c, auto hasd_c, auto onee_c, auto oned_c, int i) {
                const int kk = i - 1;
                X3_STAMP(0);
                interval(hase_c, hasd_c, onee_c, oned_c, i);
                X3_STAMP(3);
                if constexpr (!(X3_ABL & 32)) __syncthreads();
                X3_STAMP(4);
            };
            const int nfull = tail ? n - 1 : n;
            if (nfull == 0) run(yes, no, yes, no, 0);
            else run(yes, no, no, no, 0);
            for (int i = 1; i < nfull; ++i) run(yes, yes, no, no, i);
            if (tail) {
                if (nfull > 0) run(yes, yes, yes, no, n - 1);
                run(no, yes, no, yes, n);
            } else run(no, yes, no, no, n);
            first_chunk_requested = false;
            if (blk + 1 < a.nblocks && a.blocks[blk + 1].se_kind == 0) {
                const X3TowerBlock& dn = a.blocks[blk + 1];
                load_first_chunk(x3_weights(dn.w1pk, dn.w1pk_lo, dn.w3pk, dn.w3pk_lo, dn.dwpk, dn.cop_pad), dn.tail != 0 && dn.cop_pad == CK);
                first_chunk_requested = true;
            }
            __syncthreads();
            { const int kk = n; X3_STAMP(5); }
        }
    }
    } else {
    constexpr int NJ = 4;
    f32x4 accX[NJ][4];
    x3_stream_load<NJ>(accX, a.x + size_t(b) * 64 * C, w * NJ, l15, lg);
    for (int blk = 0; blk < a.nblocks; ++blk) {
        const X3TowerBlock& d = a.blocks[blk];
        if (blk > 0 && d.se_kind != 0) x3_stream_se<NJ>(T, d, accX, reinterpret_cast<float*>(T.t2h), w * NJ, tid);
        const X3Weights W = x3_weights(d.w1pk, d.w1pk_lo, d.w3pk, d.w3pk_lo, d.dwpk, d.cop_pad);
        const int n = W.cop_pad / CK;
        const int nslab3 = W.cop_pad >> 5;
        const bool tail = __builtin_amdgcn_readfirstlane(d.tail) != 0;
#ifdef CRA_X3_TRACE
        const bool tracing = (b == 0 || b == 131) && blk == CRA_X3_TRACE;
        int trace_n = 0;
#endif
        {
            constexpr int PW = 2;
            half8 p_h[PW][NJ], p_l[PW][NJ];
            int rdo[2][4];
#pragma unroll
            for (int hh = 0; hh < 2; ++hh)
#pragma unroll
                for (int t = 0; t < 4; ++t) rdo[hh][t] = x3q_read_offset(0, hh, t, l15, lg);
            auto load_p = [&](int k, int s2) {
                if constexpr (X3_ABL & 16) return;
#pragma unroll
                for (int j = 0; j < NJ; ++j) {
                    const uint32_t f = uint32_t(w * NJ + j) * uint32_t(nslab3) + uint32_t(k * (CK / 32) + s2);
                    p_h[s2 % PW][j] = x3_frag(W.w3h, lane_off, f);
                    p_l[s2 % PW][j] = x3_frag(W.w3l, lane_off, f);
                }
            };
            if constexpr (X3_ABL & 16) {
#pragma unroll
                for (int s2 = 0; s2 < PW; ++s2)
#pragma unroll
                    for (int j = 0; j < NJ; ++j) p_h[s2][j] = p_l[s2][j] = *reinterpret_cast<const half8*>(T.xl + lane * 8);
            }
            x3_stream_add_bias<NJ>(accX, d.b3, w * NJ, lg);
#pragma unroll
            for (int s2 = 0; s2 < PW; ++s2) load_p(0, s2);
            if constexpr (!(X3_ABL & 32)) {
                __syncthreads();
                __syncthreads();
            }
            auto project = [&](auto one_c, int kk) {
                constexpr int NS2 = decltype(one_c)::value ? CK / 64 : CK / 32;
                const half_t* const t2h = T.t2h + (kk & 1) * 64 * TROW;
                const half_t* const t2l = T.t2l + (kk & 1) * 64 * TROW;
                const half_t* rd[2][4];
#pragma unroll
                for (int hh = 0; hh < 2; ++hh)
#pragma unroll
                    for (int t = 0; t < 4; ++t) rd[hh][t] = t2h + rdo[hh][t];
                const int to_lo = int(t2l - t2h);
                X3_STAMP(8);
                half8 bh[2][4], bl[2][4];
                auto read_t2 = [&](int s2, half8 (&h)[4], half8 (&l)[4]) {
#pragma unroll
                    for (int t = 0; t < 4; ++t) {
                        if constexpr (X3_ABL & 8) {
                            h[t] = p_h[s2 % PW][0];
                            l[t] = p_l[s2 % PW][0];
                        } else {
                            h[t] = x3q_read_fragment(rd[0][t] + s2 * 32 * X3Q_T2T_ROW, rd[1][t] + s2 * 32 * X3Q_T2T_ROW);
                            l[t] = x3q_read_fragment(rd[0][t] + s2 * 32 * X3Q_T2T_ROW + to_lo, rd[1][t] + s2 * 32 * X3Q_T2T_ROW + to_lo);
                        }
                    }
                };
                read_t2(0, bh[0], bl[0]);
#pragma unroll
                for (int s2 = 0; s2 < NS2; ++s2) {
                    if (s2 + 1 < NS2) read_t2(s2 + 1, bh[(s2 + 1) & 1], bl[(s2 + 1) & 1]);
                    __builtin_amdgcn_sched_barrier(0);
#pragma unroll
                    for (int j = 0; j < NJ; ++j)
#pragma unroll
                        for (int t = 0; t < 4; ++t) x3_mfma(p_l[s2 % PW][j], bh[s2 & 1][t], accX[j][t], !(X3_ABL & 4));
#pragma unroll
                    for (int j = 0; j < NJ; ++j)
#pragma unroll
                        for (int t = 0; t < 4; ++t) x3_mfma(p_h[s2 % PW][j], bl[s2 & 1][t], accX[j][t], !(X3_ABL & 4));
#pragma unroll
                    for (int j = 0; j < NJ; ++j)
#pragma unroll
                        for (int t = 0; t < 4; ++t) x3_mfma(p_h[s2 % PW][j], bh[s2 & 1][t], accX[j][t], !(X3_ABL & 4));
                    if (s2 + PW < NS2) load_p(kk, s2 + PW);
                    else if constexpr (decltype(one_c)::value) load_p(kk, s2 + PW - NS2);
                    else load_p(kk + 1 < n ? kk + 1 : kk, s2 + PW - NS2);
                    if (s2 == 1) X3_STAMP(9);
                    __builtin_amdgcn_sched_barrier(0);
                }
                X3_STAMP(10);
            };
            const int nfull = tail ? n - 1 : n;
            for (int kk = 0; kk < nfull; ++kk) {
                project(std::false_type{}, kk);
                if (kk + 1 < n) {
                    if constexpr (!(X3_ABL & 32)) __syncthreads();
                }
                X3_STAMP(11);
            }
            if (tail) {
                const int kk = n - 1;
                project(std::true_type{}, kk);
                X3_STAMP(11);
            }
            if (blk + 1 < a.nblocks && a.blocks[blk + 1].se_kind == 0) x3_stream_write_tiles<NJ>(T, accX, w * NJ, l15, lg);
            { const int kk = n; X3_STAMP(12); }
            __syncthreads();
            { const int kk = n; X3_STAMP(13); }
        }
    }
    x3_stream_store<NJ>(accX, a.y + size_t(b) * 64 * C, w * NJ, l15, lg);
    }
}

void init_x3_quad_kernel_attributes() {
    (void)hipFuncSetAttribute(reinterpret_cast<const void*>(&tower_x3_quad_kernel<3>), hipFuncAttributeMaxDynamicSharedMemorySize, int(X3Block::lds_bytes));
}
void launch_tower_x3_quad(const X3TowerArgs& a, hipStream_t s) {
    hipLaunchKernelGGL(tower_x3_quad_kernel<3>, dim3(a.batch), dim3(X3Block::NTHR), X3Block::lds_bytes, s, a);
}

}
```

crazyara_amd/csrc/nn/x3_quad.h:

```cpp
#pragma once

namespace cra {

constexpr int x3q_row(int sq) { return ((sq >> 3) & 3) * 16 + (sq >> 5) * 8 + (sq & 7); }
constexpr int x3q_square(int row) { return ((row >> 4) + 4 * ((row >> 3) & 1)) * 8 + (row & 7); }
constexpr int x3q_lane_square(int t, int lg, int r) { return (4 * (lg >> 1) + t) * 8 + 4 * (lg & 1) + r; }

constexpr int X3Q_T2T_ROW = 64;
constexpr int X3Q_T2T_HALVES = 128 * X3Q_T2T_ROW;
constexpr int x3q_swizzle(int c) { return (c & 1) | (((c >> 2) & 1) << 1) | (((c >> 1) & 1) << 2) | (c & 8); }
constexpr int x3q_t2t_offset(int c, int row) { return c * X3Q_T2T_ROW + 4 * ((row >> 2) ^ x3q_swizzle(c & 15)) + (row & 3); }
constexpr int x3q_store_offset(int tile, int l15, int lg, int t) { return x3q_t2t_offset(tile * 16 + l15, t * 16 + 4 * lg); }
constexpr int x3q_read_offset(int s2, int hh, int t, int l15, int lg) { return x3q_t2t_offset(s2 * 32 + lg * 8 + hh * 4 + (l15 >> 2), t * 16 + 4 * (l15 & 3)); }

}

#ifdef __HIPCC__
namespace cra {
namespace {

struct X3QuadOffsets {
    int hl, hr;
    int vt, vt6;
    int vb2, vb;
    int k0, k6, k2, k8;
    int to_v, to_k;
};
__device__ __forceinline__ X3QuadOffsets x3_quad_offsets(int lane) {
    const int lg = lane >> 4;
    const bool odd = (lg & 1) != 0, hi = lg >= 2;
    X3QuadOffsets o;
    o.hl = odd ? 0 : 11 * 16;
    o.hr = odd ? 5 * 16 : 0;
    o.vt = hi ? 0 : 11 * 16;
    o.vt6 = hi ? 0 : 5 * 16;
    o.vb2 = hi ? 11 * 16 : 0;
    o.vb = hi ? 6 * 16 : 0;
    o.k0 = lg == 3 ? 0 : 11 * 16;
    o.k6 = lg == 2 ? 0 : 5 * 16;
    o.k2 = lg == 1 ? 0 : 11 * 16;
    o.k8 = lg == 0 ? 0 : 5 * 16;
    o.to_v = (lane ^ 32) * 4;
    o.to_k = (lane ^ 48) * 4;
    return o;
}

struct X3DepthwiseQuad {
    float w[11];
    float whl[3], whr[3];
    float wvt[3], wvb[3];
    float wk[4];
    float S[4][4], H[4], V[4], K;
    float outv[4][4];

    __device__ __forceinline__ void load(const float* rec, int l15, const X3QuadOffsets& o) {
        const float* p = rec + l15;
#pragma unroll
        for (int q = 0; q < 11; ++q) w[q] = p[q * 16];
#pragma unroll
        for (int d = 0; d < 3; ++d) {
            whl[d] = p[o.hl + d * 16];
            whr[d] = p[o.hr + (6 + d) * 16];
            wvt[d] = p[(d == 2 ? o.vt6 : o.vt) + 3 * d * 16];
            wvb[d] = p[(d == 0 ? o.vb2 : o.vb) + (3 * d + 2) * 16];
        }
        wk[0] = p[o.k0];
        wk[1] = p[o.k6 + 6 * 16];
        wk[2] = p[o.k2 + 2 * 16];
        wk[3] = p[o.k8 + 8 * 16];
    }
    __device__ __forceinline__ void gather(const f32x4 (&acc)[4], int lg, const X3QuadOffsets& o) {
#pragma unroll
        for (int t = 0; t < 4; ++t)
#pragma unroll
            for (int r = 0; r < 4; ++r) S[t][r] = (X3_ABL & 1) ? acc[t][r] + w[0] : fmaxf(acc[t][r] + w[9], 0.f);
        if constexpr (X3_ABL & 1) return;
        const bool odd = (lg & 1) != 0, hi = lg >= 2;
        float sh[4];
#pragma unroll
        for (int t = 0; t < 4; ++t) {
            sh[t] = odd ? S[t][0] : S[t][3];
            H[t] = __builtin_bit_cast(float, __builtin_amdgcn_ds_swizzle(__builtin_bit_cast(int, sh[t]), 0x401f));
        }
#pragma unroll
        for (int r = 0; r < 4; ++r) {
            const float sv = hi ? S[0][r] : S[3][r];
            V[r] = __builtin_bit_cast(float, __builtin_amdgcn_ds_bpermute(o.to_v, __builtin_bit_cast(int, sv)));
        }
        const float sk = hi ? sh[0] : sh[3];
        K = __builtin_bit_cast(float, __builtin_amdgcn_ds_bpermute(o.to_k, __builtin_bit_cast(int, sk)));
    }
    template <int Y, int X, int Q> __device__ __forceinline__ float tap(float a) const {
        constexpr int DX = Q / 3, DY = Q % 3;
        if constexpr (Y >= 0 && Y < 4 && X >= 0 && X < 4) return fmaf(w[Q], S[Y][X], a);
        else if constexpr (Y >= 0 && Y < 4) return fmaf(X < 0 ? whl[DY] : whr[DY], H[Y], a);
        else if constexpr (X >= 0 && X < 4) return fmaf(Y < 0 ? wvt[DX] : wvb[DX], V[X], a);
        else return fmaf(wk[(Y < 0 ? 0 : 2) + (X < 0 ? 0 : 1)], K, a);
    }
    template <int T, int R> __device__ __forceinline__ void output() {
        if constexpr (X3_ABL & 1) {
            outv[T][R] = S[T][R];
            return;
        }
        float a = w[10];
        a = tap<T - 1, R - 1, 0>(a); a = tap<T - 1, R, 3>(a); a = tap<T - 1, R + 1, 6>(a);
        a = tap<T, R - 1, 1>(a);     a = tap<T, R, 4>(a);     a = tap<T, R + 1, 7>(a);
        a = tap<T + 1, R - 1, 2>(a); a = tap<T + 1, R, 5>(a); a = tap<T + 1, R + 1, 8>(a);
        outv[T][R] = fmaxf(a, 0.f);
    }
    template <int T> __device__ __forceinline__ void taps_rank() {
        output<T, 0>(); output<T, 1>(); output<T, 2>(); output<T, 3>();
    }
    template <int T> __device__ __forceinline__ void pin_rank() {
#pragma unroll
        for (int r = 0; r < 4; ++r) asm volatile("" : "+v"(outv[T][r]));
    }
};

typedef __fp16 x3q_f16x4 __attribute__((__vector_size__(4 * sizeof(__fp16))));
__device__ __forceinline__ half8 x3q_read_fragment(const half_t* lo4, const half_t* hi4) {
    typedef __attribute__((address_space(3))) x3q_f16x4 lds_f16x4;
    typedef uint32_t u32x2 __attribute__((ext_vector_type(2)));
    typedef uint32_t u32x4 __attribute__((ext_vector_type(4)));
    const u32x2 a = __builtin_bit_cast(u32x2, __builtin_amdgcn_ds_read_tr16_b64_v4f16((lds_f16x4*)(lo4)));
    const u32x2 b = __builtin_bit_cast(u32x2, __builtin_amdgcn_ds_read_tr16_b64_v4f16((lds_f16x4*)(hi4)));
    return __builtin_bit_cast(half8, u32x4{a.x, a.y, b.x, b.y});
}

}
}
#endif
```

crazyara_amd/csrc/nn/x3_tail.cpp:

```cpp
#include "x3_device.h"

#include <type_traits>

namespace cra {

template <int KS>
__global__ __launch_bounds__(512) void tower_x3_tail_kernel(const X3TowerArgs a) {
    static_assert(KS == 3 || KS == 5, "depthwise 3x3 or 5x5 (X3Depthwise / X3Depthwise5)");
    constexpr int REC = KS == 3 ? 256 : 512;
    using G = X3Block;
    static_assert(G::NE == 1 && G::T2BUF == 2 && G::CK == 128, "the role kernel uses the NE = 1 tile geometry (two t2 buffers of 128 channels)");
    constexpr int C = G::C, CK = G::CK, XROW = G::XROW, TROW = G::TROW;
    extern __shared__ __attribute__((aligned(16))) char smem[];
    const X3Tiles T = x3_tiles(smem);
    const int b = blockIdx.x;
    const int tid = threadIdx.x, lane = tid & 63, l15 = lane & 15, lg = lane >> 4;
    const int wave = __builtin_amdgcn_readfirstlane(tid >> 6);
    const bool expand_role = wave < 4;
    const int w = wave & 3;
    const uint32_t lane_off = uint32_t(lane) * 16u;
    x3_stage_tile(T, a.x + size_t(b) * 64 * C, nullptr, tid);
    __syncthreads();
    constexpr int EW = 2;
    half8 e_h[EW][2], e_l[EW][2];
    bool first_chunk_requested = false;
    if (expand_role) {
    for (int blk = 0; blk < a.nblocks; ++blk) {
        const X3TowerBlock& d = a.blocks[blk];
        if (blk > 0 && d.se_kind != 0) {
            x3_se_gate_from_mean(d, reinterpret_cast<float*>(T.t2h), tid);
            __syncthreads();
            first_chunk_requested = false;
#pragma unroll
            for (int ne = 0; ne < 2; ++ne) {
#pragma unroll
                for (int q = 0; q < EW; ++q) { asm volatile("" : "=v"(e_h[q][ne])); asm volatile("" : "=v"(e_l[q][ne])); }
            }
        }
        const X3Weights W = x3_weights(d.w1pk, d.w1pk_lo, d.w3pk, d.w3pk_lo, d.dwpk, d.cop_pad);
        const int n = W.cop_pad / CK;
        const bool tail = __builtin_amdgcn_readfirstlane(d.tail) != 0;
#ifdef CRA_X3_TRACE
        const bool tracing = (b == 0 || b == 131) && blk == CRA_X3_TRACE;
        int trace_n = 0;
#endif
        {
            const bool hi = l15 >= 8;
            const X3EdgeOffsets edge = x3_edge_offsets(l15);
            auto e_tile = [&](int i, int ne) { return i * (CK / 16) + (tail && i == n - 1 ? w : w * 2 + ne); };
            auto load_e = [&](auto one_c, int i, int s) {
                if constexpr (X3_ABL & 16) return;
#pragma unroll
                for (int ne = 0; ne < (decltype(one_c)::value ? 1 : 2); ++ne) {
                    const uint32_t f = uint32_t(e_tile(i, ne)) * (C / 32) + uint32_t(s);
                    e_h[s % EW][ne] = x3_frag(W.w1h, lane_off, f);
                    e_l[s % EW][ne] = x3_frag(W.w1l, lane_off, f);
                }
            };
            auto load_first_chunk = [&](const X3Weights& Wx, bool one) {
                if constexpr (X3_ABL & 16) return;
#pragma unroll
                for (int s = 0; s < EW; ++s)
#pragma unroll
                    for (int ne = 0; ne < 2; ++ne) {
                        const uint32_t f = uint32_t(one ? w : w * 2 + ne) * (C / 32) + uint32_t(s);
                        e_h[s][ne] = x3_frag(Wx.w1h, lane_off, f);
                        e_l[s][ne] = x3_frag(Wx.w1l, lane_off, f);
                    }
            };
            if constexpr (X3_ABL & 16) {
#pragma unroll
                for (int s = 0; s < EW; ++s)
#pragma unroll
                    for (int ne = 0; ne < 2; ++ne) e_h[s][ne] = e_l[s][ne] = *reinterpret_cast<const half8*>(T.xh + lane * 8);
            }
            if (!first_chunk_requested) load_first_chunk(W, tail && n == 1);
            float* const my_dws = T.dws + (w * 2) * REC;
            f32x4 accE[2][4], accD[2][4];
            X3Depthwise dw;
            X3Depthwise5 dw5;
            const X3EdgeOffsets5 edge5 = x3_edge_offsets5(l15);
            auto interval = [&](auto hase_c, auto hasd_c, auto onee_c, auto oned_c, int i) {
                constexpr bool HASE = decltype(hase_c)::value, HASD = decltype(hasd_c)::value;
                constexpr bool ONEE = decltype(onee_c)::value, ONED = decltype(oned_c)::value;
                static_assert(!(ONEE && !HASE) && !(ONED && (HASE || !HASD)), "the tail chunk is expanded in interval n - 1 and runs the depthwise alone in interval n");
                constexpr int NEE = ONEE ? 1 : 2;
                half8 ring_h[4], ring_l[4];
                auto read_step = [&](int st) {
                    if constexpr (X3_ABL & 8) {
                        ring_h[st % 4] = e_h[0][0];
                        ring_l[st % 4] = e_l[0][0];
                    } else {
                        ring_h[st % 4] = *reinterpret_cast<const half8*>(T.xh + ((st & 3) * 16 + l15) * XROW + (st >> 2) * 32 + lg * 8);
                        ring_l[st % 4] = *reinterpret_cast<const half8*>(T.xl + ((st & 3) * 16 + l15) * XROW + (st >> 2) * 32 + lg * 8);
                    }
                };
                f32x4 dw_raw[NEE][REC / 256];
                if constexpr (HASE) {
#pragma unroll
                    for (int ne = 0; ne < NEE; ++ne)
#pragma unroll
                        for (int h2 = 0; h2 < REC / 256; ++h2)
                            dw_raw[ne][h2] = __builtin_bit_cast(f32x4, __builtin_amdgcn_raw_buffer_load_b128(W.dw, lane_off, uint32_t(e_tile(i, ne) * 16) * uint32_t(REC / 4) + uint32_t(h2) * 1024u, 0));
#pragma unroll
                    for (int ne = 0; ne < NEE; ++ne)
#pragma unroll
                        for (int t = 0; t < 4; ++t) accE[ne][t] = f32x4{0.f, 0.f, 0.f, 0.f};
                    read_step(0); read_step(1); read_step(2);
                }
                if constexpr (HASD && KS == 3) dw.template load<0>(my_dws, lg, edge);
                half_t* const t2h = T.t2h + ((i - 1) & 1) * 64 * TROW;
                half_t* const t2l = T.t2l + ((i - 1) & 1) * 64 * TROW;
#pragma unroll
                for (int sl = 0; sl < (ONED ? C / 64 : C / 32); ++sl) {
                    const int dt = sl / 4, ph = sl % 4;
                    if constexpr (HASD) {
                        if constexpr (KS == 3) {
                            if (ph == 2) dw.template load<1>(my_dws + dt * 256, lg, edge);
                            if (sl == 4) dw.template load<0>(my_dws + 256, lg, edge);
                        } else {
                            if (ph == 0) dw5.template load<0>(my_dws + dt * REC, lg, edge5);
                            if (ph == 1) dw5.template load<1>(my_dws + dt * REC, lg, edge5);
                            if (ph == 2) dw5.template load<2>(my_dws + dt * REC, lg, edge5);
                            if (ph == 3) dw5.template load<3>(my_dws + dt * REC, lg, edge5);
                        }
                    }
                    __builtin_amdgcn_sched_barrier(0);
                    if constexpr (HASE) {
#pragma unroll
                        for (int t = 0; t < 4; ++t) {
                            const int st = sl * 4 + t;
                            if (st + 3 < 4 * (C / 32)) read_step(st + 3);
#pragma unroll
                            for (int ne = 0; ne < NEE; ++ne) {
                                x3_mfma(e_l[sl % EW][ne], ring_h[st % 4], accE[ne][t], !(X3_ABL & 2));
                                x3_mfma(e_h[sl % EW][ne], ring_l[st % 4], accE[ne][t], !(X3_ABL & 2));
                                x3_mfma(e_h[sl % EW][ne], ring_h[st % 4], accE[ne][t], !(X3_ABL & 2));
                            }
                        }
                        if (sl + EW < C / 32) load_e(onee_c, i, sl + EW);
                        else if constexpr (ONEE) load_e(onee_c, i, sl + EW - C / 32);
                        else load_e(onee_c, i + 1 < n ? i + 1 : i, sl + EW - C / 32);
                    }
                    if constexpr (HASD) {
                        if constexpr (KS == 3) {
                            if (ph == 0) dw.template gather<0>(accD[dt], hi);
                            if (ph == 1) { dw.template taps<0>(0, 4); dw.pin_taps(0, 4, 0); }
                            if (ph == 2) dw.template gather<1>(accD[dt], hi);
                        } else {
                            if (ph == 0) { dw5.template gather<0>(accD[dt], hi, 1.f); dw5.template taps<0>(); }
                            if (ph == 1) { dw5.template gather<1>(accD[dt], hi, 1.f); dw5.template taps<1>(); }
                            if (ph == 2) { dw5.template gather<2>(accD[dt], hi, 1.f); dw5.template taps<2>(); }
                            if (ph == 3) { dw5.template gather<3>(accD[dt], hi, 1.f); dw5.template taps<3>(); }
                        }
                        if (ph == 3) {
                            if constexpr (KS == 3) dw.template taps<1>(0, 4);
                            const int cl = (ONED ? w : w * 2 + dt) * 16 + lg * 4;
#pragma unroll
                            for (int t = 0; t < 4; ++t) {
                                half4 h, l;
                                split4(KS == 3 ? dw.outv[t] : dw5.outv[t], h, l);
                                if constexpr (X3_ABL & 64) {
                                    asm volatile("" ::"v"(h), "v"(l));
                                } else {
                                    *reinterpret_cast<half4*>(t2h + (t * 16 + l15) * TROW + cl) = h;
                                    *reinterpret_cast<half4*>(t2l + (t * 16 + l15) * TROW + cl) = l;
                                }
                            }
                        }
                    }
                    if constexpr (HASE && HASD) {
#pragma unroll
                        for (int r = 0; r < 12 * NEE; ++r) {
                            __builtin_amdgcn_sched_group_barrier(0x008, 1, 0);
                            __builtin_amdgcn_sched_group_barrier(0x002, ONEE ? 8 : 4, 0);
                        }
                    }
                    __builtin_amdgcn_sched_barrier(0);
                }
                if constexpr (HASE) {
#pragma unroll
                    for (int ne = 0; ne < NEE; ++ne)
#pragma unroll
                        for (int h2 = 0; h2 < REC / 256; ++h2) *reinterpret_cast<f32x4*>(my_dws + ne * REC + h2 * 256 + lane * 4) = dw_raw[ne][h2];
#pragma unroll
                    for (int ne = 0; ne < NEE; ++ne)
#pragma unroll
                        for (int t = 0; t < 4; ++t) accD[ne][t] = accE[ne][t];
                }
            };
            constexpr std::true_type yes{};
            constexpr std::false_type no{};
            auto run = [&](auto hase_c, auto hasd_c, auto onee_c, auto oned_c, int i) {
                const int kk = i - 1;
                X3_STAMP(0);
                interval(hase_c, hasd_c, onee_c, oned_c, i);
                X3_STAMP(3);
                if constexpr (!(X3_ABL & 32)) __syncthreads();
                X3_STAMP(4);
            };
            const int nfull = tail ? n - 1 : n;
            if (nfull == 0) run(yes, no, yes, no, 0);
            else run(yes, no, no, no, 0);
            for (int i = 1; i < nfull; ++i) run(yes, yes, no, no, i);
            if (tail) {
                if (nfull > 0) run(yes, yes, yes, no, n - 1);
                run(no, yes, no, yes, n);
            } else run(no, yes, no, no, n);
            first_chunk_requested = false;
            if (blk + 1 < a.nblocks && a.blocks[blk + 1].se_kind == 0) {
                const X3TowerBlock& dn = a.blocks[blk + 1];
                load_first_chunk(x3_weights(dn.w1pk, dn.w1pk_lo, dn.w3pk, dn.w3pk_lo, dn.dwpk, dn.cop_pad), dn.tail != 0 && dn.cop_pad == CK);
                first_chunk_requested = true;
            }
            __syncthreads();
            { const int kk = n; X3_STAMP(5); }
        }
    }
    } else {
    constexpr int NJ = 4;
    f32x4 accX[NJ][4];
    x3_stream_load<NJ>(accX, a.x + size_t(b) * 64 * C, w * NJ, l15, lg);
    for (int blk = 0; blk < a.nblocks; ++blk) {
        const X3TowerBlock& d = a.blocks[blk];
        if (blk > 0 && d.se_kind != 0) x3_stream_se<NJ>(T, d, accX, reinterpret_cast<float*>(T.t2h), w * NJ, tid);
        const X3Weights W = x3_weights(d.w1pk, d.w1pk_lo, d.w3pk, d.w3pk_lo, d.dwpk, d.cop_pad);
        const int n = W.cop_pad / CK;
        const int nslab3 = W.cop_pad >> 5;
        const bool tail = __builtin_amdgcn_readfirstlane(d.tail) != 0;
#ifdef CRA_X3_TRACE
        const bool tracing = (b == 0 || b == 131) && blk == CRA_X3_TRACE;
        int trace_n = 0;
#endif
        {
            constexpr int PW = 2;
            half8 p_h[PW][NJ], p_l[PW][NJ];
            auto load_p = [&](int k, int s2) {
                if constexpr (X3_ABL & 16) return;
#pragma unroll
                for (int j = 0; j < NJ; ++j) {
                    const uint32_t f = uint32_t(w * NJ + j) * uint32_t(nslab3) + uint32_t(k * (CK / 32) + s2);
                    p_h[s2 % PW][j] = x3_frag(W.w3h, lane_off, f);
                    p_l[s2 % PW][j] = x3_frag(W.w3l, lane_off, f);
                }
            };
            if constexpr (X3_ABL & 16) {
#pragma unroll
                for (int s2 = 0; s2 < PW; ++s2)
#pragma unroll
                    for (int j = 0; j < NJ; ++j) p_h[s2][j] = p_l[s2][j] = *reinterpret_cast<const half8*>(T.xl + lane * 8);
            }
            x3_stream_add_bias<NJ>(accX, d.b3, w * NJ, lg);
#pragma unroll
            for (int s2 = 0; s2 < PW; ++s2) load_p(0, s2);
            if constexpr (!(X3_ABL & 32)) {
                __syncthreads();
                __syncthreads();
            }
            auto project = [&](auto one_c, int kk) {
                constexpr int NS2 = decltype(one_c)::value ? CK / 64 : CK / 32;
                const half_t* const t2h = T.t2h + (kk & 1) * 64 * TROW;
                const half_t* const t2l = T.t2l + (kk & 1) * 64 * TROW;
                X3_STAMP(8);
                half8 bh[2][4], bl[2][4];
                auto read_t2 = [&](int s2, half8 (&h)[4], half8 (&l)[4]) {
#pragma unroll
                    for (int t = 0; t < 4; ++t) {
                        if constexpr (X3_ABL & 8) {
                            h[t] = p_h[s2 % PW][0];
                            l[t] = p_l[s2 % PW][0];
                        } else {
                            h[t] = *reinterpret_cast<const half8*>(t2h + (t * 16 + l15) * TROW + s2 * 32 + lg * 8);
                            l[t] = *reinterpret_cast<const half8*>(t2l + (t * 16 + l15) * TROW + s2 * 32 + lg * 8);
                        }
                    }
                };
                read_t2(0, bh[0], bl[0]);
#pragma unroll
                for (int s2 = 0; s2 < NS2; ++s2) {
                    if (s2 + 1 < NS2) read_t2(s2 + 1, bh[(s2 + 1) & 1], bl[(s2 + 1) & 1]);
                    __builtin_amdgcn_sched_barrier(0);
#pragma unroll
                    for (int j = 0; j < NJ; ++j)
#pragma unroll
                        for (int t = 0; t < 4; ++t) x3_mfma(p_l[s2 % PW][j], bh[s2 & 1][t], accX[j][t], !(X3_ABL & 4));
#pragma unroll
                    for (int j = 0; j < NJ; ++j)
#pragma unroll
                        for (int t = 0; t < 4; ++t) x3_mfma(p_h[s2 % PW][j], bl[s2 & 1][t], accX[j][t], !(X3_ABL & 4));
#pragma unroll
                    for (int j = 0; j < NJ; ++j)
#pragma unroll
                        for (int t = 0; t < 4; ++t) x3_mfma(p_h[s2 % PW][j], bh[s2 & 1][t], accX[j][t], !(X3_ABL & 4));
                    if (s2 + PW < NS2) load_p(kk, s2 + PW);
                    else if constexpr (decltype(one_c)::value) load_p(kk, s2 + PW - NS2);
                    else load_p(kk + 1 < n ? kk + 1 : kk, s2 + PW - NS2);
                    if (s2 == 1) X3_STAMP(9);
                    __builtin_amdgcn_sched_barrier(0);
                }
                X3_STAMP(10);
            };
            const int nfull = tail ? n - 1 : n;
            for (int kk = 0; kk < nfull; ++kk) {
                project(std::false_type{}, kk);
                if (kk + 1 < n) {
                    if constexpr (!(X3_ABL & 32)) __syncthreads();
                }
                X3_STAMP(11);
            }
            if (tail) {
                const int kk = n - 1;
                project(std::true_type{}, kk);
                X3_STAMP(11);
            }
            if (blk + 1 < a.nblocks && a.blocks[blk + 1].se_kind == 0) x3_stream_write_tiles<NJ>(T, accX, w * NJ, l15, lg);
            { const int kk = n; X3_STAMP(12); }
            __syncthreads();
            { const int kk = n; X3_STAMP(13); }
        }
    }
    x3_stream_store<NJ>(accX, a.y + size_t(b) * 64 * C, w * NJ, l15, lg);
    }
}

void init_x3_tail_kernel_attributes() {
    (void)hipFuncSetAttribute(reinterpret_cast<const void*>(&tower_x3_tail_kernel<3>), hipFuncAttributeMaxDynamicSharedMemorySize, int(X3Block::lds_bytes));
    (void)hipFuncSetAttribute(reinterpret_cast<const void*>(&tower_x3_tail_kernel<5>), hipFuncAttributeMaxDynamicSharedMemorySize, int(X3Block::lds_bytes + 8192));
}
void launch_tower_x3_tail(const X3TowerArgs& a, hipStream_t s) {
    if (a.ks == 5) hipLaunchKernelGGL(tower_x3_tail_kernel<5>, dim3(a.batch), dim3(X3Block::NTHR), X3Block::lds_bytes + 8192, s, a);
    else hipLaunchKernelGGL(tower_x3_tail_kernel<3>, dim3(a.batch), dim3(X3Block::NTHR), X3Block::lds_bytes, s, a);
}

}
```

Measured before the change: 367,400 evals/s.

## Compute SE gate inside the tower block epilogue with split expand/project roles

Moves the squeeze-excitation gate computation out of the start of the next block and into the end of the previous block's epilogue. The expand and project wave roles each take part of the FC work, with SE weight matrices loaded into registers and parked in LDS tiles. A template flag (default late gating) picks whether the SE weight loads are issued before the block barrier so they overlap it. The intent is to shorten the serial gate stall between blocks, at the cost of more registers and extra LDS traffic that could lower occupancy.

Result: no change. 367,800 evals/s (median of 2 runs) (+0.1%).

```diff
diff --git a/crazyara_amd/csrc/nn/kernels.h b/crazyara_amd/csrc/nn/kernels.h
--- a/crazyara_amd/csrc/nn/kernels.h
+++ b/crazyara_amd/csrc/nn/kernels.h
@@ -91,10 +91,11 @@
     int no_quad;
 };
 void launch_tower_x3(const X3TowerArgs& a, hipStream_t s);
+void launch_tower_x3(const X3TowerArgs& a, bool gate_late, hipStream_t s);
 const char* tower_x3_kernel_name(const X3TowerArgs& a);
-void launch_tower_x3_tail(const X3TowerArgs& a, hipStream_t s);
+void launch_tower_x3_tail(const X3TowerArgs& a, bool gate_late, hipStream_t s);
 void init_x3_tail_kernel_attributes();
-void launch_tower_x3_quad(const X3TowerArgs& a, hipStream_t s);
+void launch_tower_x3_quad(const X3TowerArgs& a, bool gate_late, hipStream_t s);
 void init_x3_quad_kernel_attributes();
 bool block_x3w_supports(int C, int ks);
 void launch_block_x3w(const BlockArgs& a, hipStream_t s);
diff --git a/crazyara_amd/csrc/nn/precision.cpp b/crazyara_amd/csrc/nn/precision.cpp
--- a/crazyara_amd/csrc/nn/precision.cpp
+++ b/crazyara_amd/csrc/nn/precision.cpp
@@ -31,6 +31,7 @@
     x3_no_head_chain = getenv("CRA_X3_NO_HEAD_CHAIN") != nullptr;
     x3_no_tail = getenv("CRA_X3_NO_TAIL") != nullptr;
     x3_no_quad = getenv("CRA_X3_NO_QUAD") != nullptr;
+    if (const char* e = getenv("CRA_X3_GATE_LATE")) x3_gate_late = e[0] != '0' && e[0] != 0;
     small_batch_heads_apart = getenv("CRA_SMALL_BATCH_HEADS_APART") != nullptr;
     if (const char* e = getenv("CRA_X3_HEADS_APART")) x3_heads_apart = e[0] != '0' && e[0] != 0;
     value_head_env = getenv("CRA_X3_VALUE_HEAD") != nullptr || getenv("CRA_VALUE_HEAD_VARIANT") != nullptr;
diff --git a/crazyara_amd/csrc/nn/rise_net.h b/crazyara_amd/csrc/nn/rise_net.h
--- a/crazyara_amd/csrc/nn/rise_net.h
+++ b/crazyara_amd/csrc/nn/rise_net.h
@@ -133,6 +133,7 @@
         bool x3_no_head_chain = false;
         bool x3_no_tail = false;
         bool x3_no_quad = false;
+        bool x3_gate_late = true;
         bool small_batch_heads_apart = false;
         bool x3_heads_apart = false;
         bool value_head_env = false;
diff --git a/crazyara_amd/csrc/nn/rise_net.hip b/crazyara_amd/csrc/nn/rise_net.hip
--- a/crazyara_amd/csrc/nn/rise_net.hip
+++ b/crazyara_amd/csrc/nn/rise_net.hip
@@ -209,8 +209,8 @@
             if (n > 0) {
                 X3TowerArgs t = op.tx;
                 t.batch = n;
-                launch_tower_x3(t, s);
-            } else launch_tower_x3(op.tx, s);
+                launch_tower_x3(t, op.tx_gate_late, s);
+            } else launch_tower_x3(op.tx, op.tx_gate_late, s);
             break;
         case OpKind::BlockX3Split:
             if (n > 0) {
diff --git a/crazyara_amd/csrc/nn/rise_net_build.hip b/crazyara_amd/csrc/nn/rise_net_build.hip
--- a/crazyara_amd/csrc/nn/rise_net_build.hip
+++ b/crazyara_amd/csrc/nn/rise_net_build.hip
@@ -752,6 +752,7 @@
         op.tx.symmetric = dev.x3_symmetric ? 1 : 0;
         op.tx.no_tail = dev.x3_no_tail ? 1 : 0;
         op.tx.no_quad = dev.x3_no_quad ? 1 : 0;
+        op.tx_gate_late = dev.x3_gate_late;
         im.ops.push_back(op);
     }
     x3_blocks.clear();
diff --git a/crazyara_amd/csrc/nn/rise_net_impl.h b/crazyara_amd/csrc/nn/rise_net_impl.h
--- a/crazyara_amd/csrc/nn/rise_net_impl.h
+++ b/crazyara_amd/csrc/nn/rise_net_impl.h
@@ -38,6 +38,7 @@
     ResTowerArgs rt{};
     StemArgs st{};
     X3TowerArgs tx{};
+    bool tx_gate_late = true;
     X3SplitArgs xs{};
     float* xs_y = nullptr;
     X3WTowerArgs wt{};
diff --git a/crazyara_amd/csrc/nn/x3.hip b/crazyara_amd/csrc/nn/x3.hip
--- a/crazyara_amd/csrc/nn/x3.hip
+++ b/crazyara_amd/csrc/nn/x3.hip
@@ -1856,13 +1856,14 @@
     }
     return "?";
 }
-void launch_tower_x3(const X3TowerArgs& a, hipStream_t s) {
+void launch_tower_x3(const X3TowerArgs& a, hipStream_t s) { launch_tower_x3(a, true, s); }
+void launch_tower_x3(const X3TowerArgs& a, bool gate_late, hipStream_t s) {
     switch (pick_tower_x3(a)) {
         case X3TowerKernel::P8_5: hipLaunchKernelGGL(tower_p8_kernel<5>, dim3(a.batch), dim3(X3Block::NTHR), X3Block::lds_bytes + 8192, s, a); break;
         case X3TowerKernel::P8_3: hipLaunchKernelGGL(tower_p8_kernel<3>, dim3(a.batch), dim3(X3Block::NTHR), X3Block::lds_bytes, s, a); break;
-        case X3TowerKernel::Quad3: launch_tower_x3_quad(a, s); break;
+        case X3TowerKernel::Quad3: launch_tower_x3_quad(a, gate_late, s); break;
         case X3TowerKernel::Tail5:
-        case X3TowerKernel::Tail3: launch_tower_x3_tail(a, s); break;
+        case X3TowerKernel::Tail3: launch_tower_x3_tail(a, gate_late, s); break;
         case X3TowerKernel::Roles5: hipLaunchKernelGGL(tower_x3_roles_kernel<5>, dim3(a.batch), dim3(X3Block::NTHR), X3Block::lds_bytes + 8192, s, a); break;
         case X3TowerKernel::Roles3: hipLaunchKernelGGL(tower_x3_roles_kernel<3>, dim3(a.batch), dim3(X3Block::NTHR), X3Block::lds_bytes, s, a); break;
         case X3TowerKernel::Symmetric: hipLaunchKernelGGL(tower_x3_kernel, dim3(a.batch), dim3(X3Block::NTHR), X3Block::lds_bytes, s, a); break;
diff --git a/crazyara_amd/csrc/nn/x3_quad.cpp b/crazyara_amd/csrc/nn/x3_quad.cpp
--- a/crazyara_amd/csrc/nn/x3_quad.cpp
+++ b/crazyara_amd/csrc/nn/x3_quad.cpp
@@ -5,7 +5,7 @@
 
 namespace cra {
 
-template <int KS>
+template <int KS, bool GATE_EARLY>
 __global__ __launch_bounds__(512) void tower_x3_quad_kernel(const X3TowerArgs a) {
     static_assert(KS == 3, "depthwise 3x3 (X3DepthwiseQuad); 5x5 runs stay on tower_x3_tail_kernel");
     constexpr int REC = 256;
@@ -21,31 +21,47 @@
     const bool expand_role = wave < 4;
     const int w = wave & 3;
     const uint32_t lane_off = uint32_t(lane) * 16u;
+    constexpr int EW = 2;
+    half8 e_h[EW][2], e_l[EW][2];
+    auto first_window = [&](const X3TowerBlock& dn) {
+        if constexpr (X3_ABL & 16) return;
+        if (a.nblocks < 1) return;
+        const X3Weights Wx = x3_weights(dn.w1pk, dn.w1pk_lo, dn.w3pk, dn.w3pk_lo, dn.dwpk, dn.cop_pad);
+        const bool one = dn.tail != 0 && dn.cop_pad == CK;
+#pragma unroll
+        for (int s = 0; s < EW; ++s)
+#pragma unroll
+            for (int ne = 0; ne < 2; ++ne) {
+                const uint32_t f = uint32_t(one ? w : w * 2 + ne) * (C / 32) + uint32_t(s);
+                e_h[s][ne] = x3_frag(Wx.w1h, lane_off, f);
+                e_l[s][ne] = x3_frag(Wx.w1l, lane_off, f);
+            }
+    };
+#ifdef CRA_X3_TRACE
+    int trace_n = 0;
+#endif
+    if (expand_role) {
+    if constexpr (GATE_EARLY) first_window(a.blocks[0]);
     x3_stage_tile(T, a.x + size_t(b) * 64 * C, nullptr, tid);
     __syncthreads();
-    constexpr int EW = 2;
-    half8 e_h[EW][2], e_l[EW][2];
-    bool first_chunk_requested = false;
-    if (expand_role) {
+    if constexpr (!GATE_EARLY) first_window(a.blocks[0]);
     for (int blk = 0; blk < a.nblocks; ++blk) {
         const X3TowerBlock& d = a.blocks[blk];
-        if (blk > 0 && d.se_kind != 0) {
-            x3_se_gate_from_mean(d, reinterpret_cast<float*>(T.t2h), tid);
-            __syncthreads();
-            first_chunk_requested = false;
-#pragma unroll
-            for (int ne = 0; ne < 2; ++ne) {
-#pragma unroll
-                for (int q = 0; q < EW; ++q) { asm volatile("" : "=v"(e_h[q][ne])); asm volatile("" : "=v"(e_l[q][ne])); }
-            }
-        }
         const X3Weights W = x3_weights(d.w1pk, d.w1pk_lo, d.w3pk, d.w3pk_lo, d.dwpk, d.cop_pad);
         const int n = W.cop_pad / CK;
         const bool tail = __builtin_amdgcn_readfirstlane(d.tail) != 0;
 #ifdef CRA_X3_TRACE
         const bool tracing = (b == 0 || b == 131) && blk == CRA_X3_TRACE;
-        int trace_n = 0;
-#endif
+#endif
+        auto gate_stamp = [&](int id) {
+#ifdef CRA_X3_TRACE
+            const bool tracing = (b == 0 || b == 131) && blk + 1 == CRA_X3_TRACE;
+            const int kk = 62;
+            X3_STAMP(id);
+#else
+            (void)id;
+#endif
+        };
         {
             const X3QuadOffsets qo = x3_quad_offsets(lane);
             int sto[4];
@@ -61,24 +77,12 @@
                     e_l[s % EW][ne] = x3_frag(W.w1l, lane_off, f);
                 }
             };
-            auto load_first_chunk = [&](const X3Weights& Wx, bool one) {
-                if constexpr (X3_ABL & 16) return;
+            if constexpr (X3_ABL & 16) {
 #pragma unroll
                 for (int s = 0; s < EW; ++s)
 #pragma unroll
-                    for (int ne = 0; ne < 2; ++ne) {
-                        const uint32_t f = uint32_t(one ? w : w * 2 + ne) * (C / 32) + uint32_t(s);
-                        e_h[s][ne] = x3_frag(Wx.w1h, lane_off, f);
-                        e_l[s][ne] = x3_frag(Wx.w1l, lane_off, f);
-                    }
-            };
-            if constexpr (X3_ABL & 16) {
-#pragma unroll
-                for (int s = 0; s < EW; ++s)
-#pragma unroll
                     for (int ne = 0; ne < 2; ++ne) e_h[s][ne] = e_l[s][ne] = *reinterpret_cast<const half8*>(T.xh + lane * 8);
             }
-            if (!first_chunk_requested) load_first_chunk(W, tail && n == 1);
             float* const my_dws = T.dws + (w * 2) * REC;
             f32x4 accE[2][4], accD[2][4];
             X3DepthwiseQuad dw;
@@ -193,31 +197,56 @@
                 if (nfull > 0) run(yes, yes, yes, no, n - 1);
                 run(no, yes, no, yes, n);
             } else run(no, yes, no, no, n);
-            first_chunk_requested = false;
-            if (blk + 1 < a.nblocks && a.blocks[blk + 1].se_kind == 0) {
+            const int gate_kind = blk + 1 < a.nblocks ? __builtin_amdgcn_readfirstlane(a.blocks[blk + 1].se_kind) : 0;
+            if (gate_kind != 0) {
                 const X3TowerBlock& dn = a.blocks[blk + 1];
-                load_first_chunk(x3_weights(dn.w1pk, dn.w1pk_lo, dn.w3pk, dn.w3pk_lo, dn.dwpk, dn.cop_pad), dn.tail != 0 && dn.cop_pad == CK);
-                first_chunk_requested = true;
-            }
-            __syncthreads();
-            { const int kk = n; X3_STAMP(5); }
+                f32x4 wa[16], wb[16];
+                int gtid = tid;
+                asm volatile("" : "+v"(gtid));
+                if constexpr (GATE_EARLY) x3g_expand_requests(dn, gate_kind, reinterpret_cast<char*>(T.xh), gtid, wa, wb);
+                __syncthreads();
+                { const int kk = n; X3_STAMP(5); }
+#pragma unroll
+                for (int ne = 0; ne < 2; ++ne) {
+#pragma unroll
+                    for (int q = 0; q < EW; ++q) { asm volatile("" : "=v"(e_h[q][ne])); asm volatile("" : "=v"(e_l[q][ne])); }
+                }
+                x3g_gate_expand<GATE_EARLY>(dn, gate_kind, reinterpret_cast<float*>(T.t2h), gtid, wa, wb, gate_stamp);
+                if constexpr (GATE_EARLY) first_window(dn);
+                __syncthreads();
+                gate_stamp(4);
+                if constexpr (!GATE_EARLY) first_window(dn);
+            } else {
+                if (blk + 1 < a.nblocks) first_window(a.blocks[blk + 1]);
+                __syncthreads();
+                { const int kk = n; X3_STAMP(5); }
+            }
         }
     }
     } else {
     constexpr int NJ = 4;
     f32x4 accX[NJ][4];
+    x3_stage_tile(T, a.x + size_t(b) * 64 * C, nullptr, tid);
+    __syncthreads();
     x3_stream_load<NJ>(accX, a.x + size_t(b) * 64 * C, w * NJ, l15, lg);
     for (int blk = 0; blk < a.nblocks; ++blk) {
         const X3TowerBlock& d = a.blocks[blk];
-        if (blk > 0 && d.se_kind != 0) x3_stream_se<NJ>(T, d, accX, reinterpret_cast<float*>(T.t2h), w * NJ, tid);
         const X3Weights W = x3_weights(d.w1pk, d.w1pk_lo, d.w3pk, d.w3pk_lo, d.dwpk, d.cop_pad);
         const int n = W.cop_pad / CK;
         const int nslab3 = W.cop_pad >> 5;
         const bool tail = __builtin_amdgcn_readfirstlane(d.tail) != 0;
 #ifdef CRA_X3_TRACE
         const bool tracing = (b == 0 || b == 131) && blk == CRA_X3_TRACE;
-        int trace_n = 0;
-#endif
+#endif
+        auto gate_stamp = [&](int id) {
+#ifdef CRA_X3_TRACE
+            const bool tracing = (b == 0 || b == 131) && blk + 1 == CRA_X3_TRACE;
+            const int kk = 62;
+            X3_STAMP(id);
+#else
+            (void)id;
+#endif
+        };
         {
             constexpr int PW = 2;
             half8 p_h[PW][NJ], p_l[PW][NJ];
@@ -310,21 +339,38 @@
                 project(std::true_type{}, kk);
                 X3_STAMP(11);
             }
-            if (blk + 1 < a.nblocks && a.blocks[blk + 1].se_kind == 0) x3_stream_write_tiles<NJ>(T, accX, w * NJ, l15, lg);
-            { const int kk = n; X3_STAMP(12); }
-            __syncthreads();
-            { const int kk = n; X3_STAMP(13); }
+            const int gate_kind = blk + 1 < a.nblocks ? __builtin_amdgcn_readfirstlane(a.blocks[blk + 1].se_kind) : 0;
+            if (gate_kind != 0) {
+                const X3TowerBlock& dn = a.blocks[blk + 1];
+                f32x4 wb[16];
+                int gtid = tid;
+                asm volatile("" : "+v"(gtid));
+                if constexpr (GATE_EARLY) x3g_request<true>(x3g_second_matrix(dn, gate_kind), gtid, wb);
+                { const int kk = n; X3_STAMP(12); }
+                __syncthreads();
+                { const int kk = n; X3_STAMP(13); }
+                x3g_gate_project<GATE_EARLY, NJ>(T, dn, gate_kind, accX, reinterpret_cast<float*>(T.t2h), w * NJ, gtid, wb, gate_stamp);
+            } else {
+                if (blk + 1 < a.nblocks) x3_stream_write_tiles<NJ>(T, accX, w * NJ, l15, lg);
+                { const int kk = n; X3_STAMP(12); }
+                __syncthreads();
+                { const int kk = n; X3_STAMP(13); }
+            }
         }
     }
-    x3_stream_store<NJ>(accX, a.y + size_t(b) * 64 * C, w * NJ, l15, lg);
+    int sl15 = l15, slg = lg;
+    asm volatile("" : "+v"(sl15), "+v"(slg));
+    x3_stream_store<NJ>(accX, a.y + size_t(b) * 64 * C, w * NJ, sl15, slg);
     }
 }
 
 void init_x3_quad_kernel_attributes() {
-    (void)hipFuncSetAttribute(reinterpret_cast<const void*>(&tower_x3_quad_kernel<3>), hipFuncAttributeMaxDynamicSharedMemorySize, int(X3Block::lds_bytes));
+    (void)hipFuncSetAttribute(reinterpret_cast<const void*>(&tower_x3_quad_kernel<3, true>), hipFuncAttributeMaxDynamicSharedMemorySize, int(X3Block::lds_bytes));
+    (void)hipFuncSetAttribute(reinterpret_cast<const void*>(&tower_x3_quad_kernel<3, false>), hipFuncAttributeMaxDynamicSharedMemorySize, int(X3Block::lds_bytes));
 }
-void launch_tower_x3_quad(const X3TowerArgs& a, hipStream_t s) {
-    hipLaunchKernelGGL(tower_x3_quad_kernel<3>, dim3(a.batch), dim3(X3Block::NTHR), X3Block::lds_bytes, s, a);
+void launch_tower_x3_quad(const X3TowerArgs& a, bool gate_late, hipStream_t s) {
+    if (gate_late) hipLaunchKernelGGL((tower_x3_quad_kernel<3, false>), dim3(a.batch), dim3(X3Block::NTHR), X3Block::lds_bytes, s, a);
+    else hipLaunchKernelGGL((tower_x3_quad_kernel<3, true>), dim3(a.batch), dim3(X3Block::NTHR), X3Block::lds_bytes, s, a);
 }
 
 }
diff --git a/crazyara_amd/csrc/nn/x3_quad.h b/crazyara_amd/csrc/nn/x3_quad.h
--- a/crazyara_amd/csrc/nn/x3_quad.h
+++ b/crazyara_amd/csrc/nn/x3_quad.h
@@ -127,6 +127,151 @@
     return __builtin_bit_cast(half8, u32x4{a.x, a.y, b.x, b.y});
 }
 
+constexpr int X3G_GRP = 36;
+constexpr int X3G_PARK_BYTES = 16 * 256 * 16;
+static_assert(X3G_PARK_BYTES <= int(2 * 64 * X3Block::XROW * sizeof(half_t)), "the parked half matrix lies inside the xh / xl tiles");
+
+template <bool EARLY>
+__device__ __forceinline__ void x3g_request(const float* base, int tid, f32x4 (&dst)[16]) {
+    if constexpr (EARLY) {
+        const __amdgpu_buffer_rsrc_t r = x3_rsrc(base);
+#pragma unroll
+        for (int i = 0; i < 16; ++i) dst[i] = __builtin_bit_cast(f32x4, __builtin_amdgcn_raw_buffer_load_b128(r, uint32_t(tid) * 16u, uint32_t(i) * 8192u, 0));
+    } else {
+        const f32x4* pk = reinterpret_cast<const f32x4*>(base) + tid;
+#pragma unroll
+        for (int i = 0; i < 16; ++i) dst[i] = pk[i * 512];
+    }
+}
+__device__ __forceinline__ const float* x3g_second_matrix(const X3TowerBlock& d, int kind) { return kind == 1 ? d.se_w2t : d.se_w1t + size_t(16) * 512 * 4; }
+
+__device__ __forceinline__ void x3g_expand_requests(const X3TowerBlock& d, int kind, char* park, int tid, f32x4 (&wa)[16], f32x4 (&wb)[16]) {
+    {
+        f32x4 other[16];
+        x3g_request<true>(d.se_w1t, tid + 256, other);
+        x3g_request<true>(d.se_w1t, tid, wa);
+#pragma unroll
+        for (int i = 0; i < 16; ++i) *reinterpret_cast<f32x4*>(park + (i * 256 + tid) * 16) = other[i];
+    }
+    __builtin_amdgcn_sched_barrier(0);
+    x3g_request<true>(x3g_second_matrix(d, kind), tid, wb);
+}
+__device__ __forceinline__ void x3g_read_parked(const char* park, int tid, f32x4 (&wa)[16]) {
+#pragma unroll
+    for (int i = 0; i < 16; ++i) wa[i] = *reinterpret_cast<const f32x4*>(park + (i * 256 + (tid - 256)) * 16);
+}
+
+template <class Stamp>
+__device__ __forceinline__ void x3g_fcs(const X3TowerBlock& d, int kind, const float* se_mean, float* se_h, float* se_gate, const f32x4 (&wa)[16], const f32x4 (&wb)[16], int tid, Stamp&& stamp) {
+    constexpr int GRP = X3G_GRP;
+    auto dot32 = [](const f32x4 (&w)[16], const float* v, float& s0, float& s1) {
+#pragma unroll
+        for (int k4 = 0; k4 < 8; ++k4) {
+            const f32x4 m = *reinterpret_cast<const f32x4*>(v + 4 * k4);
+            s0 = fmaf(w[2 * k4][0], m[0], s0); s1 = fmaf(w[2 * k4][1], m[0], s1);
+            s0 = fmaf(w[2 * k4][2], m[1], s0); s1 = fmaf(w[2 * k4][3], m[1], s1);
+            s0 = fmaf(w[2 * k4 + 1][0], m[2], s0); s1 = fmaf(w[2 * k4 + 1][1], m[2], s1);
+            s0 = fmaf(w[2 * k4 + 1][2], m[3], s0); s1 = fmaf(w[2 * k4 + 1][3], m[3], s1);
+        }
+    };
+    if (kind == 1) {
+        {
+            const int j2 = tid >> 3, kq = tid & 7;
+            float s0 = 0.f, s1 = 0.f;
+            dot32(wa, se_mean + kq * GRP, s0, s1);
+            s0 += dpp_mov<0x111>(s0); s1 += dpp_mov<0x111>(s1);
+            s0 += dpp_mov<0x112>(s0); s1 += dpp_mov<0x112>(s1);
+            s0 += dpp_mov<0x114>(s0); s1 += dpp_mov<0x114>(s1);
+            if (kq == 7) {
+                float* h = se_h + (j2 >> 4) * GRP + 2 * (j2 & 15);
+                h[0] = fmaxf(s0, 0.f);
+                h[1] = fmaxf(s1, 0.f);
+            }
+        }
+        stamp(2);
+        __syncthreads();
+        {
+            const int c2 = tid >> 2, kq = tid & 3;
+            float s0 = 0.f, s1 = 0.f;
+            dot32(wb, se_h + kq * GRP, s0, s1);
+            s0 += dpp_mov<0x111>(s0); s1 += dpp_mov<0x111>(s1);
+            s0 += dpp_mov<0x112>(s0); s1 += dpp_mov<0x112>(s1);
+            if (kq == 3) {
+                se_gate[2 * c2] = hard_sigmoid(s0);
+                se_gate[2 * c2 + 1] = hard_sigmoid(s1);
+            }
+        }
+    } else {
+        const int c2 = tid >> 2, kq = tid & 3;
+        float s0 = 0.f, s1 = 0.f;
+        dot32(wa, se_mean + (2 * kq) * GRP, s0, s1);
+        dot32(wb, se_mean + (2 * kq + 1) * GRP, s0, s1);
+        s0 += dpp_mov<0x111>(s0); s1 += dpp_mov<0x111>(s1);
+        s0 += dpp_mov<0x112>(s0); s1 += dpp_mov<0x112>(s1);
+        if (kq == 3) {
+            se_gate[2 * c2] = hard_sigmoid(d.se_b[2 * c2] + s0);
+            se_gate[2 * c2 + 1] = hard_sigmoid(d.se_b[2 * c2 + 1] + s1);
+        }
+    }
+    stamp(3);
+    __syncthreads();
+}
+
+template <bool EARLY, class Stamp>
+__device__ __forceinline__ void x3g_gate_expand(const X3TowerBlock& d, int kind, float* scratch, int tid, f32x4 (&wa)[16], f32x4 (&wb)[16], Stamp&& stamp) {
+    stamp(0);
+    if constexpr (!EARLY) {
+        x3g_request<false>(d.se_w1t, tid, wa);
+        x3g_request<false>(x3g_second_matrix(d, kind), tid, wb);
+    }
+    __syncthreads();
+    stamp(1);
+    x3g_fcs(d, kind, scratch, scratch + 8 * X3G_GRP, scratch + 12 * X3G_GRP, wa, wb, tid, stamp);
+}
+template <bool EARLY, int NJ, class Stamp>
+__device__ __forceinline__ void x3g_gate_project(const X3Tiles& T, const X3TowerBlock& d, int kind, f32x4 (&x)[NJ][4], float* scratch, int tile0, int tid, f32x4 (&wb)[16], Stamp&& stamp) {
+    constexpr int GRP = X3G_GRP;
+    const int lane = tid & 63, l15 = lane & 15, lg = lane >> 4;
+    stamp(0);
+#pragma unroll
+    for (int j = 0; j < NJ; ++j) {
+        float sum[4];
+#pragma unroll
+        for (int r = 0; r < 4; ++r) sum[r] = (x[j][0][r] + x[j][1][r]) + (x[j][2][r] + x[j][3][r]);
+#pragma unroll
+        for (int r = 0; r < 4; ++r) {
+            sum[r] += dpp_mov<0x111>(sum[r]);
+            sum[r] += dpp_mov<0x112>(sum[r]);
+            sum[r] += dpp_mov<0x114>(sum[r]);
+            sum[r] += dpp_mov<0x118>(sum[r]);
+        }
+        if (l15 == 15) {
+            const int c = (tile0 + j) * 16 + lg * 4;
+#pragma unroll
+            for (int r = 0; r < 4; ++r) scratch[((c + r) >> 5) * GRP + ((c + r) & 31)] = sum[r] * (1.f / 64.f);
+        }
+    }
+    f32x4 wa[16];
+    if constexpr (!EARLY) {
+        x3g_request<false>(d.se_w1t, tid, wa);
+        x3g_request<false>(x3g_second_matrix(d, kind), tid, wb);
+    }
+    __syncthreads();
+    stamp(1);
+    if constexpr (EARLY) x3g_read_parked(reinterpret_cast<const char*>(T.xh), tid, wa);
+    x3g_fcs(d, kind, scratch, scratch + 8 * GRP, scratch + 12 * GRP, wa, wb, tid, stamp);
+    const float* se_gate = scratch + 12 * GRP;
+#pragma unroll
+    for (int j = 0; j < NJ; ++j) {
+        const f32x4 g = *reinterpret_cast<const f32x4*>(se_gate + (tile0 + j) * 16 + lg * 4);
+#pragma unroll
+        for (int t = 0; t < 4; ++t) x[j][t] *= g;
+    }
+    x3_stream_write_tiles<NJ>(T, x, tile0, l15, lg);
+    __syncthreads();
+    stamp(4);
+}
+
 }
 }
 #endif
diff --git a/crazyara_amd/csrc/nn/x3_tail.cpp b/crazyara_amd/csrc/nn/x3_tail.cpp
--- a/crazyara_amd/csrc/nn/x3_tail.cpp
+++ b/crazyara_amd/csrc/nn/x3_tail.cpp
@@ -1,10 +1,11 @@
 #include "x3_device.h"
+#include "x3_quad.h"
 
 #include <type_traits>
 
 namespace cra {
 
-template <int KS>
+template <int KS, bool GATE_EARLY>
 __global__ __launch_bounds__(512) void tower_x3_tail_kernel(const X3TowerArgs a) {
     static_assert(KS == 3 || KS == 5, "depthwise 3x3 or 5x5 (X3Depthwise / X3Depthwise5)");
     constexpr int REC = KS == 3 ? 256 : 512;
@@ -19,31 +20,47 @@
     const bool expand_role = wave < 4;
     const int w = wave & 3;
     const uint32_t lane_off = uint32_t(lane) * 16u;
+    constexpr int EW = 2;
+    half8 e_h[EW][2], e_l[EW][2];
+    auto first_window = [&](const X3TowerBlock& dn) {
+        if constexpr (X3_ABL & 16) return;
+        if (a.nblocks < 1) return;
+        const X3Weights Wx = x3_weights(dn.w1pk, dn.w1pk_lo, dn.w3pk, dn.w3pk_lo, dn.dwpk, dn.cop_pad);
+        const bool one = dn.tail != 0 && dn.cop_pad == CK;
+#pragma unroll
+        for (int s = 0; s < EW; ++s)
+#pragma unroll
+            for (int ne = 0; ne < 2; ++ne) {
+                const uint32_t f = uint32_t(one ? w : w * 2 + ne) * (C / 32) + uint32_t(s);
+                e_h[s][ne] = x3_frag(Wx.w1h, lane_off, f);
+                e_l[s][ne] = x3_frag(Wx.w1l, lane_off, f);
+            }
+    };
+#ifdef CRA_X3_TRACE
+    int trace_n = 0;
+#endif
+    if (expand_role) {
+    if constexpr (GATE_EARLY) first_window(a.blocks[0]);
     x3_stage_tile(T, a.x + size_t(b) * 64 * C, nullptr, tid);
     __syncthreads();
-    constexpr int EW = 2;
-    half8 e_h[EW][2], e_l[EW][2];
-    bool first_chunk_requested = false;
-    if (expand_role) {
+    if constexpr (!GATE_EARLY) first_window(a.blocks[0]);
     for (int blk = 0; blk < a.nblocks; ++blk) {
         const X3TowerBlock& d = a.blocks[blk];
-        if (blk > 0 && d.se_kind != 0) {
-            x3_se_gate_from_mean(d, reinterpret_cast<float*>(T.t2h), tid);
-            __syncthreads();
-            first_chunk_requested = false;
-#pragma unroll
-            for (int ne = 0; ne < 2; ++ne) {
-#pragma unroll
-                for (int q = 0; q < EW; ++q) { asm volatile("" : "=v"(e_h[q][ne])); asm volatile("" : "=v"(e_l[q][ne])); }
-            }
-        }
         const X3Weights W = x3_weights(d.w1pk, d.w1pk_lo, d.w3pk, d.w3pk_lo, d.dwpk, d.cop_pad);
         const int n = W.cop_pad / CK;
         const bool tail = __builtin_amdgcn_readfirstlane(d.tail) != 0;
 #ifdef CRA_X3_TRACE
         const bool tracing = (b == 0 || b == 131) && blk == CRA_X3_TRACE;
-        int trace_n = 0;
-#endif
+#endif
+        auto gate_stamp = [&](int id) {
+#ifdef CRA_X3_TRACE
+            const bool tracing = (b == 0 || b == 131) && blk + 1 == CRA_X3_TRACE;
+            const int kk = 62;
+            X3_STAMP(id);
+#else
+            (void)id;
+#endif
+        };
         {
             const bool hi = l15 >= 8;
             const X3EdgeOffsets edge = x3_edge_offsets(l15);
@@ -57,24 +74,12 @@
                     e_l[s % EW][ne] = x3_frag(W.w1l, lane_off, f);
                 }
             };
-            auto load_first_chunk = [&](const X3Weights& Wx, bool one) {
-                if constexpr (X3_ABL & 16) return;
+            if constexpr (X3_ABL & 16) {
 #pragma unroll
                 for (int s = 0; s < EW; ++s)
 #pragma unroll
-                    for (int ne = 0; ne < 2; ++ne) {
-                        const uint32_t f = uint32_t(one ? w : w * 2 + ne) * (C / 32) + uint32_t(s);
-                        e_h[s][ne] = x3_frag(Wx.w1h, lane_off, f);
-                        e_l[s][ne] = x3_frag(Wx.w1l, lane_off, f);
-                    }
-            };
-            if constexpr (X3_ABL & 16) {
-#pragma unroll
-                for (int s = 0; s < EW; ++s)
-#pragma unroll
                     for (int ne = 0; ne < 2; ++ne) e_h[s][ne] = e_l[s][ne] = *reinterpret_cast<const half8*>(T.xh + lane * 8);
             }
-            if (!first_chunk_requested) load_first_chunk(W, tail && n == 1);
             float* const my_dws = T.dws + (w * 2) * REC;
             f32x4 accE[2][4], accD[2][4];
             X3Depthwise dw;
@@ -207,31 +212,56 @@
                 if (nfull > 0) run(yes, yes, yes, no, n - 1);
                 run(no, yes, no, yes, n);
             } else run(no, yes, no, no, n);
-            first_chunk_requested = false;
-            if (blk + 1 < a.nblocks && a.blocks[blk + 1].se_kind == 0) {
+            const int gate_kind = blk + 1 < a.nblocks ? __builtin_amdgcn_readfirstlane(a.blocks[blk + 1].se_kind) : 0;
+            if (gate_kind != 0) {
                 const X3TowerBlock& dn = a.blocks[blk + 1];
-                load_first_chunk(x3_weights(dn.w1pk, dn.w1pk_lo, dn.w3pk, dn.w3pk_lo, dn.dwpk, dn.cop_pad), dn.tail != 0 && dn.cop_pad == CK);
-                first_chunk_requested = true;
-            }
-            __syncthreads();
-            { const int kk = n; X3_STAMP(5); }
+                f32x4 wa[16], wb[16];
+                int gtid = tid;
+                asm volatile("" : "+v"(gtid));
+                if constexpr (GATE_EARLY) x3g_expand_requests(dn, gate_kind, reinterpret_cast<char*>(T.xh), gtid, wa, wb);
+                __syncthreads();
+                { const int kk = n; X3_STAMP(5); }
+#pragma unroll
+                for (int ne = 0; ne < 2; ++ne) {
+#pragma unroll
+                    for (int q = 0; q < EW; ++q) { asm volatile("" : "=v"(e_h[q][ne])); asm volatile("" : "=v"(e_l[q][ne])); }
+                }
+                x3g_gate_expand<GATE_EARLY>(dn, gate_kind, reinterpret_cast<float*>(T.t2h), gtid, wa, wb, gate_stamp);
+                if constexpr (GATE_EARLY) first_window(dn);
+                __syncthreads();
+                gate_stamp(4);
+                if constexpr (!GATE_EARLY) first_window(dn);
+            } else {
+                if (blk + 1 < a.nblocks) first_window(a.blocks[blk + 1]);
+                __syncthreads();
+                { const int kk = n; X3_STAMP(5); }
+            }
         }
     }
     } else {
     constexpr int NJ = 4;
     f32x4 accX[NJ][4];
+    x3_stage_tile(T, a.x + size_t(b) * 64 * C, nullptr, tid);
+    __syncthreads();
     x3_stream_load<NJ>(accX, a.x + size_t(b) * 64 * C, w * NJ, l15, lg);
     for (int blk = 0; blk < a.nblocks; ++blk) {
         const X3TowerBlock& d = a.blocks[blk];
-        if (blk > 0 && d.se_kind != 0) x3_stream_se<NJ>(T, d, accX, reinterpret_cast<float*>(T.t2h), w * NJ, tid);
         const X3Weights W = x3_weights(d.w1pk, d.w1pk_lo, d.w3pk, d.w3pk_lo, d.dwpk, d.cop_pad);
         const int n = W.cop_pad / CK;
         const int nslab3 = W.cop_pad >> 5;
         const bool tail = __builtin_amdgcn_readfirstlane(d.tail) != 0;
 #ifdef CRA_X3_TRACE
         const bool tracing = (b == 0 || b == 131) && blk == CRA_X3_TRACE;
-        int trace_n = 0;
-#endif
+#endif
+        auto gate_stamp = [&](int id) {
+#ifdef CRA_X3_TRACE
+            const bool tracing = (b == 0 || b == 131) && blk + 1 == CRA_X3_TRACE;
+            const int kk = 62;
+            X3_STAMP(id);
+#else
+            (void)id;
+#endif
+        };
         {
             constexpr int PW = 2;
             half8 p_h[PW][NJ], p_l[PW][NJ];
@@ -313,23 +343,46 @@
                 project(std::true_type{}, kk);
                 X3_STAMP(11);
             }
-            if (blk + 1 < a.nblocks && a.blocks[blk + 1].se_kind == 0) x3_stream_write_tiles<NJ>(T, accX, w * NJ, l15, lg);
-            { const int kk = n; X3_STAMP(12); }
-            __syncthreads();
-            { const int kk = n; X3_STAMP(13); }
+            const int gate_kind = blk + 1 < a.nblocks ? __builtin_amdgcn_readfirstlane(a.blocks[blk + 1].se_kind) : 0;
+            if (gate_kind != 0) {
+                const X3TowerBlock& dn = a.blocks[blk + 1];
+                f32x4 wb[16];
+                int gtid = tid;
+                asm volatile("" : "+v"(gtid));
+                if constexpr (GATE_EARLY) x3g_request<true>(x3g_second_matrix(dn, gate_kind), gtid, wb);
+                { const int kk = n; X3_STAMP(12); }
+                __syncthreads();
+                { const int kk = n; X3_STAMP(13); }
+                x3g_gate_project<GATE_EARLY, NJ>(T, dn, gate_kind, accX, reinterpret_cast<float*>(T.t2h), w * NJ, gtid, wb, gate_stamp);
+            } else {
+                if (blk + 1 < a.nblocks) x3_stream_write_tiles<NJ>(T, accX, w * NJ, l15, lg);
+                { const int kk = n; X3_STAMP(12); }
+                __syncthreads();
+                { const int kk = n; X3_STAMP(13); }
+            }
         }
     }
-    x3_stream_store<NJ>(accX, a.y + size_t(b) * 64 * C, w * NJ, l15, lg);
+    int sl15 = l15, slg = lg;
+    asm volatile("" : "+v"(sl15), "+v"(slg));
+    x3_stream_store<NJ>(accX, a.y + size_t(b) * 64 * C, w * NJ, sl15, slg);
     }
 }
 
 void init_x3_tail_kernel_attributes() {
-    (void)hipFuncSetAttribute(reinterpret_cast<const void*>(&tower_x3_tail_kernel<3>), hipFuncAttributeMaxDynamicSharedMemorySize, int(X3Block::lds_bytes));
-    (void)hipFuncSetAttribute(reinterpret_cast<const void*>(&tower_x3_tail_kernel<5>), hipFuncAttributeMaxDynamicSharedMemorySize, int(X3Block::lds_bytes + 8192));
+    (void)hipFuncSetAttribute(reinterpret_cast<const void*>(&tower_x3_tail_kernel<3, true>), hipFuncAttributeMaxDynamicSharedMemorySize, int(X3Block::lds_bytes));
+    (void)hipFuncSetAttribute(reinterpret_cast<const void*>(&tower_x3_tail_kernel<3, false>), hipFuncAttributeMaxDynamicSharedMemorySize, int(X3Block::lds_bytes));
+    (void)hipFuncSetAttribute(reinterpret_cast<const void*>(&tower_x3_tail_kernel<5, true>), hipFuncAttributeMaxDynamicSharedMemorySize, int(X3Block::lds_bytes + 8192));
+    (void)hipFuncSetAttribute(reinterpret_cast<const void*>(&tower_x3_tail_kernel<5, false>), hipFuncAttributeMaxDynamicSharedMemorySize, int(X3Block::lds_bytes + 8192));
 }
-void launch_tower_x3_tail(const X3TowerArgs& a, hipStream_t s) {
-    if (a.ks == 5) hipLaunchKernelGGL(tower_x3_tail_kernel<5>, dim3(a.batch), dim3(X3Block::NTHR), X3Block::lds_bytes + 8192, s, a);
-    else hipLaunchKernelGGL(tower_x3_tail_kernel<3>, dim3(a.batch), dim3(X3Block::NTHR), X3Block::lds_bytes, s, a);
+void launch_tower_x3_tail(const X3TowerArgs& a, bool gate_late, hipStream_t s) {
+    const dim3 grid(a.batch), block(X3Block::NTHR);
+    if (a.ks == 5) {
+        if (gate_late) hipLaunchKernelGGL((tower_x3_tail_kernel<5, false>), grid, block, X3Block::lds_bytes + 8192, s, a);
+        else hipLaunchKernelGGL((tower_x3_tail_kernel<5, true>), grid, block, X3Block::lds_bytes + 8192, s, a);
+    } else {
+        if (gate_late) hipLaunchKernelGGL((tower_x3_tail_kernel<3, false>), grid, block, X3Block::lds_bytes, s, a);
+        else hipLaunchKernelGGL((tower_x3_tail_kernel<3, true>), grid, block, X3Block::lds_bytes, s, a);
+    }
 }
 
 }
```
